# gergely-flamich/compression-without-quantization

Measured on AMD Instinct MI355X. Metric: latent blocks encoded/s at KL=16 bits, higher is better.
Workload: dtype f32

## Files before the change

### compression_without_quantization_amd/_lib.py

```python
import ctypes
import os

_HERE = os.path.dirname(os.path.abspath(__file__))
LIB_PATH = os.environ.get("CWQ_LIB_PATH") or os.path.join(_HERE, "libcwq.so")

c_int = ctypes.c_int
c_i32 = ctypes.c_int32
c_i64 = ctypes.c_int64
c_f32 = ctypes.c_float
c_f64 = ctypes.c_double
c_size = ctypes.c_size_t
c_vp = ctypes.c_void_p
c_str = ctypes.c_char_p


class Options(ctypes.Structure):
    _fields_ = [("prune_mode", ctypes.c_int32), ("reserved", ctypes.c_int32),
                ("eval_start_event", c_vp), ("eval_stop_event", c_vp),
                ("eval_ms_out", ctypes.POINTER(ctypes.c_float)),
                ("item_ready", c_vp)]


c_opts = ctypes.POINTER(Options)

# ... 22 lines not shown
                                          c_i32, c_f32, c_i64, c_vp, c_vp, c_vp, c_size, c_opts,
                                          c_vp]),
    "cwq_greedy_decode": (c_int, [c_vp, c_vp, c_vp, c_vp, c_i64, c_i64, c_i64, c_int, c_int,
                                  c_i32, c_f32, c_i64, c_vp, c_vp]),
    "cwq_greedy_decode_uniform": (c_int, [c_vp, c_vp, c_vp, c_i64, c_i64, c_int, c_int, c_i32,
                                          c_f32, c_i64, c_vp, c_vp]),
    "cwq_block_bits": (c_int, [c_vp, c_vp, c_vp, c_vp, c_i64, c_i64, c_f64, c_int, c_int, c_vp,
                               c_vp, c_vp]),
    "cwq_greedy_encode_uniform_var_workspace_size": (c_size, [c_i64, c_i64]),
    "cwq_greedy_encode_uniform_var": (c_int, [c_vp, c_vp, c_vp, c_vp, c_i64, c_i64, c_vp, c_int,
                                              c_i32, c_f32, c_i64, c_vp, c_vp, c_vp, c_size,
                                              c_opts, c_vp]),
    "cwq_block_bits_csr": (c_int, [c_vp, c_vp, c_vp, c_vp, c_vp, c_i64, c_i64, c_f64, c_int,
                                   c_int, c_int, c_vp, c_vp, c_vp]),
    "cwq_greedy_encode_var_workspace_size": (c_size, [c_i64, c_i64, c_i64, c_int]),
    "cwq_greedy_encode_var": (c_int, [c_vp, c_vp, c_vp, c_vp, c_vp, c_i64, c_i64, c_i64, c_vp,
                                      c_int, c_i32, c_f32, c_i64, c_vp, c_vp, c_vp, c_size,
                                      c_opts, c_vp]),
    "cwq_pack_indices_var_workspace_size": (c_size, [c_i64]),
    "cwq_pack_indices_var": (c_int, [c_vp, c_vp, c_i64, c_int, c_vp, c_i64, c_vp, c_vp, c_size,
                                     c_vp]),
    "cwq_unpack_indices_var": (c_int, [c_vp, c_i64, c_vp, c_i64, c_int, c_vp, c_vp, c_size,
                                       c_vp]),
    "cwq_standardise": (c_int, [c_vp, c_vp, c_vp, c_vp, c_i64, c_vp, c_vp, c_vp]),
    "cwq_kl_normal_normal": (c_int, [c_vp, c_vp, c_vp, c_vp, c_i64, c_vp, c_vp]),
    "cwq_destandardise": (c_int, [c_vp, c_vp, c_vp, c_i64, c_vp, c_vp]),
    "cwq_group_starts": (c_i64, [c_vp, c_i64, c_i64, c_f64, c_vp, c_i64]),
    "cwq_code_grouped_greedy_workspace_size": (c_size, [c_i64, c_int]),
    "cwq_code_grouped_greedy": (c_i64, [c_vp, c_vp, c_vp, c_vp, c_i64, c_int, c_int, c_i32, c_f32,
                                        c_i64, c_f64, c_vp, c_vp, c_i64, c_vp, c_i64, c_vp, c_vp,
                                        c_size, c_opts, c_vp]),
    "cwq_code_grouped_greedy_begin": (c_i64, [c_vp, c_vp, c_vp, c_vp, c_i64, c_int, c_int, c_i32,
                                              c_f32, c_i64, c_f64, c_vp, c_vp, c_i64, c_vp, c_i64,
                                              c_vp, c_vp, c_size, c_opts, c_vp]),
    "cwq_code_grouped_greedy_end": (c_i64, [c_vp, c_i64, c_int, c_int, c_vp, c_i64, c_vp]),
    "cwq_code_grouped_greedy_batch_workspace_size": (c_size, [c_i64, c_i64, c_int]),
    "cwq_code_grouped_greedy_batch_host_workspace_size": (c_size, [c_i64, c_i64, c_int]),
    "cwq_code_grouped_greedy_batch": (c_i64, [c_i64, c_vp, c_vp, c_vp, c_vp, c_vp, c_int, c_int,
                                              c_vp, c_f32, c_i64, c_f64, c_vp, c_vp, c_i64, c_vp,
                                              c_vp, c_i64, c_vp, c_vp, c_size, c_vp, c_size,
                                              c_opts, c_vp]),
    "cwq_importance_workspace_size": (c_size, [c_i64, c_i64]),
    "cwq_importance_encode": (c_int, [c_vp, c_vp, c_vp, c_vp, c_vp, c_vp, c_i64, c_i64, c_i32,
                                      c_i64, c_vp, c_vp, c_vp, c_size, c_opts, c_vp]),
    "cwq_importance_decode": (c_int, [c_vp, c_vp, c_vp, c_vp, c_i64, c_i64, c_i32, c_i64, c_vp,
                                      c_vp]),
    "cwq_importance_group_starts": (c_i64, [c_vp, c_i64, c_i64, c_f64, c_vp, c_i64]),
    "cwq_importance_plan": (c_int, [c_vp, c_vp, c_i64, c_vp]),
    "cwq_code_grouped_importance_workspace_size": (c_size, [c_i64]),
    "cwq_code_grouped_importance": (c_i64, [c_vp, c_vp, c_vp, c_vp, c_i64, c_i32, c_f32, c_i64,
                                            c_f64, c_vp, c_vp, c_vp, c_i64, c_vp, c_vp, c_vp,
                                            c_vp, c_vp, c_size, c_opts, c_vp]),
    "cwq_code_grouped_importance_batch_workspace_size": (c_size, [c_i64, c_i64]),
    "cwq_code_grouped_importance_batch": (c_i64, [c_i64, c_vp, c_vp, c_vp, c_vp, c_vp, c_vp,
                                                  c_f32, c_i64, c_f64, c_vp, c_vp, c_vp, c_i64,
                                                  c_vp, c_vp, c_vp, c_vp, c_vp, c_vp, c_size,
                                                  c_opts, c_vp]),
    "cwq_decode_grouped_greedy_batch_workspace_size": (c_size, [c_i64, c_i64, c_int]),
    "cwq_decode_grouped_greedy_batch_host_workspace_size": (c_size, [c_i64, c_i64, c_int]),
    "cwq_decode_grouped_greedy_batch": (c_i64, [c_i64, c_vp, c_vp, c_vp, c_vp, c_vp, c_vp, c_vp,
                                                c_int, c_int, c_vp, c_f32, c_vp, c_vp, c_vp,
                                                c_size, c_vp, c_size, c_opts, c_vp]),
    "cwq_decode_grouped_importance_batch_workspace_size": (c_size, [c_i64, c_i64]),
    "cwq_decode_grouped_importance_batch_host_workspace_size": (c_size, [c_i64, c_i64]),
    "cwq_decode_grouped_importance_batch": (c_i64, [c_i64, c_vp, c_vp, c_vp, c_vp, c_vp, c_vp,
                                                    c_vp, c_vp, c_vp, c_vp, c_vp, c_size, c_vp,
                                                    c_size, c_opts, c_vp]),
    "cwq_ac_encode": (c_i64, [c_vp, c_i64, c_int, c_vp, c_i64, c_vp, c_i64]),
    "cwq_ac_decode": (c_i64, [c_vp, c_i64, c_int, c_vp, c_i64, c_vp, c_i64]),
    "cwq_elias_delta_encode": (c_i64, [c_vp, c_i64, c_vp, c_i64]),
    "cwq_elias_delta_decode": (c_i64, [c_vp, c_i64, c_i64, c_vp]),
    "cwq_bitcode_to_indices": (c_i64, [c_vp, c_i64, c_int, c_i64, c_vp]),
    "cwq_selftest_bm_tables": (c_int, [ctypes.c_uint32, c_i64, c_vp, c_vp, c_vp, c_vp]),
    "cwq_selftest_screen_tables": (c_int, [ctypes.c_uint32, c_i64, c_vp, c_vp, c_vp, c_vp]),
    "cwq_selftest_logf": (c_int, [c_vp, c_i64, c_vp, c_vp]),
    "cwq_selftest_wave_max": (c_int, [c_vp, c_i64, c_vp, c_vp]),
    "cwq_selftest_div": (c_int, [c_vp, c_vp, c_i64, c_vp, c_vp]),
    "cwq_selftest_encode_rows_wave": (c_int, [c_vp, c_vp, c_vp, c_vp, c_vp, c_i64, c_i64, c_i64,
                                              c_int, c_int, c_i32, c_f32, c_i64, c_vp, c_vp, c_vp,
                                              c_size, c_vp]),
    "cwq_selftest_encode_uniform_tau_guess": (c_int, [c_vp, c_vp, c_vp, c_vp, c_i64, c_i64, c_int,
                                                      c_int, c_i32, c_f32, c_i64, c_vp, c_vp, c_vp,
                                                      c_size, c_opts, c_vp, c_int]),
    "cwq_beam_encode_workspace_size": (c_size, [c_i64, c_i64, c_i64, c_int, c_int]),
    "cwq_beam_encode": (c_int, [c_vp, c_vp, c_vp, c_vp, c_vp, c_i64, c_i64, c_i64, c_int, c_int,
                                c_int, c_i32, c_f32, c_i64, c_vp, c_vp, c_vp, c_vp, c_size, c_opts,
                                c_vp]),
    "cwq_selftest_beam_encode": (c_int, [c_vp, c_vp, c_vp, c_vp, c_vp, c_i64, c_i64, c_i64, c_int,
                                         c_int, c_int, c_i32, c_f32, c_i64, c_vp, c_vp, c_vp, c_vp,
                                         c_size, c_opts, c_vp, c_int]),
    "cwq_beam_encode_var": (c_int, [c_vp, c_vp, c_vp, c_vp, c_vp, c_i64, c_i64, c_i64, c_vp, c_int,
                                    c_int, c_int, c_i32, c_f32, c_i64, c_vp, c_vp, c_vp, c_vp,
                                    c_size, c_opts, c_vp]),
    "cwq_selftest_beam_encode_var": (c_int, [c_vp, c_vp, c_vp, c_vp, c_vp, c_i64, c_i64, c_i64,
                                             c_vp, c_int, c_int, c_int, c_i32, c_f32, c_i64, c_vp,
                                             c_vp, c_vp, c_vp, c_size, c_opts, c_vp, c_int]),
    "cwq_greedy_backfit_workspace_size": (c_size, [c_i64, c_i64, c_i64, c_int]),
    "cwq_greedy_backfit": (c_int, [c_vp, c_vp, c_vp, c_vp, c_vp, c_i64, c_i64, c_i64, c_int, c_int,
                                   c_int, c_i32, c_f32, c_i64, c_vp, c_vp, c_vp, c_vp, c_vp, c_size,
                                   c_opts, c_vp]),
    "cwq_greedy_backfit_var": (c_int, [c_vp, c_vp, c_vp, c_vp, c_vp, c_i64, c_i64, c_i64, c_vp,
                                       c_int, c_int, c_i32, c_f32, c_i64, c_vp, c_vp, c_vp, c_vp,
                                       c_vp, c_size, c_opts, c_vp]),
    "cwq_pln_posterior": (c_int, [c_vp, c_vp, c_vp, c_vp, c_i64, c_f32, c_vp, c_vp, c_vp]),
    "cwq_permute_gather": (c_int, [c_vp, c_i64, c_i64, c_vp, c_vp, c_vp]),
    "cwq_permute_scatter": (c_int, [c_vp, c_i64, c_i64, c_vp, c_vp, c_vp]),
}

TOOL_SIGNATURES = {
    "cwq_debug_prune_stats": (c_int, [c_vp, c_int]),
    "cwq_debug_tile_times": (c_int, [c_vp, c_vp, c_vp, c_int]),
    "cwq_debug_quad_times": (c_int, [c_vp, c_vp, c_int]),
    "cwq_debug_partition_workspace_size": (c_size, [c_i64]),
    "cwq_debug_group_starts_device": (c_i64, [c_vp, c_i64, c_i64, c_f64, c_vp, c_vp, c_size,
                                              c_vp, c_vp]),
}

ABI_VERSION = (0 << 16) | 15

_lib = None


class CwqError(RuntimeError):
    """A libcwq call returned an error code."""


def load():
    global _lib
    if _lib is not None:
        return _lib
    if not os.path.exists(LIB_PATH):
        raise ImportError(
            f"{LIB_PATH} not found: build the HIP extension first "
            "(python -c 'import __graft_entry__ as g; g.build()')")
    lib = ctypes.CDLL(LIB_PATH)
    lib.cwq_version.restype = c_int
    lib.cwq_version.argtypes = []
    ver = lib.cwq_version()
    if ver != ABI_VERSION:
        raise ImportError(f"{LIB_PATH} has ABI version {ver >> 16}.{ver & 0xffff}, these "
                          f"bindings need {ABI_VERSION >> 16}.{ABI_VERSION & 0xffff}: rebuild it")
    for name, (res, args) in list(SIGNATURES.items()) + list(TOOL_SIGNATURES.items()):
        if not hasattr(lib, name):
            if name in TOOL_SIGNATURES:
                continue
            raise ImportError(f"{LIB_PATH} does not export {name}: rebuild it")
        fn = getattr(lib, name)
        fn.restype = res
        fn.argtypes = args
    _lib = lib
    return lib


def check(rc, what):
    if rc < 0:
        msg = load().cwq_last_error().decode("utf-8", "replace")
        raise CwqError(f"{what} failed ({rc}): {msg}")
    return rc
```

### compression_without_quantization_amd/coded_greedy_sampler.py

```python
import array
import concurrent.futures
import ctypes
import functools
import threading
import warnings
import weakref
import time

import numpy as np
import torch

from . import _lib
from .binary_io import bitcode_to_indices, indices_to_bitcode

VERBOSE = True


def _device_of(*xs):
    for x in xs:
        if isinstance(x, torch.Tensor) and x.is_cuda:
            return x.device
    if not torch.cuda.is_available():
        raise RuntimeError("compression_without_quantization_amd needs a ROCm GPU "
                           "(torch.cuda.is_available() is False); there is no CPU path")
    return torch.device("cuda", torch.cuda.current_device())


def _is_float32(x):
    if isinstance(x, torch.Tensor):
        return x.dtype == torch.float32
    return np.asarray(x).dtype == np.float32


def _f32(x, device, what):
    if isinstance(x, torch.Tensor):
        if x.device == device and x.dtype == torch.float32 and x.is_contiguous():
            return x.view(-1)
        t = x
    else:
        t = torch.from_numpy(np.ascontiguousarray(np.asarray(x)))
    if t.dtype != torch.float32:
        raise TypeError(f"{what} must be float32, got {t.dtype}")
    return t.to(device=device).contiguous().reshape(-1)


def _ptr(t):
    return t.data_ptr() if t is not None and t.numel() > 0 else None


def _like_input(t, ref):
    if isinstance(ref, torch.Tensor):
        return t
    return t.cpu().numpy()


class Normal:

    def __init__(self, loc, scale):
        self.loc = loc
        self.scale = scale

    @property
    def dtype(self):
        return self.loc.dtype


def encode_workspace_bytes(nb, total_dims, block_dim=None, max_block_dim=None):
    lib = _lib.load()
    if block_dim is not None:
        return int(lib.cwq_greedy_encode_uniform_workspace_size(int(nb), int(block_dim)))
    mbd = int(total_dims if max_block_dim is None else max_block_dim)
    return int(lib.cwq_greedy_encode_workspace_size(int(nb), int(total_dims), mbd))


def encode_blocks(t_loc, t_scale, p_loc, p_scale, n_bits_per_step, n_steps, seed, rho=1.,
                  block_dim=None, block_off=None, max_block_dim=None, block_id_base=0,
                  out_idx=None, out_sample=None, workspace=None, prune_mode=None,
                  eval_events=None):
    lib = _lib.load()
    dev = _device_of(t_loc, t_scale, p_loc, p_scale)
    tl = _f32(t_loc, dev, "t_loc")
    ts = _f32(t_scale, dev, "t_scale")
    pl = _f32(p_loc, dev, "p_loc")
    ps = _f32(p_scale, dev, "p_scale")
    D = tl.numel()
    if not (ts.numel() == pl.numel() == ps.numel() == D):
        raise ValueError("t_loc, t_scale, p_loc, p_scale must have the same size")
    if (block_dim is None) == (block_off is None):
        raise ValueError("give exactly one of block_dim / block_off")
    if block_dim is not None:
        block_dim = int(block_dim)
        if block_dim < 0 or (block_dim == 0 and D != 0) or (block_dim and D % block_dim):
            raise ValueError(f"D={D} is not a multiple of block_dim={block_dim}")
        nb = D // block_dim if block_dim else 0
        offs = None
    else:
        offs_h = np.asarray(block_off.cpu() if isinstance(block_off, torch.Tensor)
                            else block_off, dtype=np.int64).reshape(-1)
        nb = offs_h.size - 1
        if nb < 0 or offs_h[0] != 0 or offs_h[-1] != D or (np.diff(offs_h) < 0).any():
            raise ValueError("block_off must be non-decreasing from 0 to D")
        if max_block_dim is None:
            max_block_dim = int(np.diff(offs_h).max()) if nb > 0 else 0
        offs = torch.from_numpy(offs_h).to(dev)
    n_steps = int(n_steps)
    if out_idx is None:
        out_idx = torch.empty((nb, n_steps), dtype=torch.int32, device=dev)
    if out_sample is None:
        out_sample = torch.empty(D, dtype=torch.float32, device=dev)
    need = encode_workspace_bytes(nb, D, block_dim if offs is None else None,
                                  None if offs is None else max_block_dim)
    if workspace is None or workspace.numel() < need:
        workspace = torch.empty(max(need, 1), dtype=torch.uint8, device=dev)
    opts = _lib.options(prune_mode, eval_events)
    seed32 = int(np.int32(np.uint32(int(seed) & 0xFFFFFFFF)))
    with torch.cuda.device(dev):
        stream = torch.cuda.current_stream(dev).cuda_stream
        if offs is None:
            rc = lib.cwq_greedy_encode_uniform(
                _ptr(tl), _ptr(ts), _ptr(pl), _ptr(ps), nb, block_dim, int(n_bits_per_step),
                n_steps, seed32, float(rho), int(block_id_base), _ptr(out_idx),
                _ptr(out_sample), workspace.data_ptr(), workspace.numel(), opts, stream)
        else:
            rc = lib.cwq_greedy_encode(
                _ptr(tl), _ptr(ts), _ptr(pl), _ptr(ps), offs.data_ptr(), nb, D,
                int(max_block_dim), int(n_bits_per_step), n_steps, seed32, float(rho),
                int(block_id_base), _ptr(out_idx), _ptr(out_sample), workspace.data_ptr(),
                workspace.numel(), opts, stream)
    _lib.check(rc, "cwq_greedy_encode")
    return out_idx, out_sample


def decode_blocks(idx, p_loc, p_scale, n_bits_per_step, n_steps, seed, rho=1.,
                  block_dim=None, block_off=None, block_id_base=0, out_sample=None):
    lib = _lib.load()
    dev = _device_of(idx, p_loc, p_scale)
    pl = _f32(p_loc, dev, "p_loc")
    ps = _f32(p_scale, dev, "p_scale")
    D = pl.numel()
    if ps.numel() != D:
        raise ValueError("p_loc and p_scale must have the same size")
    it = idx if isinstance(idx, torch.Tensor) else torch.from_numpy(np.asarray(idx))
    it = it.to(device=dev, dtype=torch.int32).contiguous().reshape(-1)
    n_steps = int(n_steps)
    if out_sample is None:
        out_sample = torch.empty(D, dtype=torch.float32, device=dev)
    stream = torch.cuda.current_stream(dev).cuda_stream
    seed32 = int(np.int32(np.uint32(int(seed) & 0xFFFFFFFF)))
    if (block_dim is None) == (block_off is None):
        raise ValueError("give exactly one of block_dim / block_off")
    with torch.cuda.device(dev):
        return _decode_blocks_on(lib, it, pl, ps, D, n_steps, n_bits_per_step, seed32, rho,
                                 block_dim, block_off, block_id_base, out_sample, dev, stream)
# ... 573 lines not shown
```

### compression_without_quantization_amd/csrc/cwq_capi.hip

```cpp
#include <hip/hip_runtime.h>
#include <hsa/hsa.h>
#include <hsa/hsa_ext_amd.h>
#include <stdint.h>
#include <stdarg.h>
#include <stdio.h>
#include <math.h>
#include <string.h>
#include <time.h>
#include <immintrin.h>

#include <algorithm>
#include <atomic>
#include <memory>
#include <condition_variable>
#include <functional>
#include <mutex>
#include <sched.h>
#include <unistd.h>
#include <stdlib.h>
#include <thread>
#include <vector>

#include "../../include/cwq.h"
#include "cwq_debug.h"
// ... 192 lines not shown
      }
    }
  }
  starts[ns++] = D - 1;
  starts[ns++] = D;
  ok();
  return ns;
}

int read_options(const cwq_options* opts, cwq_options* out) {
  const cwq_options def = CWQ_OPTIONS_INIT;
  *out = opts ? *opts : def;
  if (out->prune_mode < 0 || out->prune_mode > 2)
    return fail(CWQ_ERR_INVALID, "cwq_options.prune_mode=%d outside [0, 2]", out->prune_mode);
  if (out->reserved != 0) return fail(CWQ_ERR_INVALID, "cwq_options.reserved must be 0");
  if ((out->eval_start_event == nullptr) != (out->eval_stop_event == nullptr))
    return fail(CWQ_ERR_INVALID, "cwq_options: give both eval events or neither");
  return CWQ_OK;
}

int check_common(int n_bits, int n_steps, int64_t nb) {
  if (n_bits < 0 || n_bits > CWQ_MAX_BITS_PER_STEP)
    return fail(CWQ_ERR_INVALID, "n_bits_per_step=%d outside [0, %d]", n_bits,
                CWQ_MAX_BITS_PER_STEP);
  if (n_steps < 1) return fail(CWQ_ERR_INVALID, "n_steps=%d must be >= 1", n_steps);
  if (nb < 0) return fail(CWQ_ERR_INVALID, "nb=%lld must be >= 0", (long long)nb);
  return CWQ_OK;
}

void fill_encode_args(cwq::EncodeArgs& a, const float* t_loc, const float* t_scale,
                      const float* p_loc, const float* p_scale, const int64_t* block_off,
                      int64_t ud, int64_t nb, int64_t total_dims, int64_t max_d, int n_bits,
                      int n_steps, int32_t seed, float rho, int64_t block_id_base,
                      int32_t* out_idx, float* out_sample, const cwq_options& o,
                      const cwq::EncWs& l, void* w) {
  a.t_loc = t_loc;
  a.t_scale = t_scale;
  a.p_loc = p_loc;
  a.p_scale = p_scale;
  a.block_off = block_off;
  a.ud = ud;
  a.nb = nb;
  a.total_dims = total_dims;
  a.max_d = max_d;
  a.n_cand = (int64_t)1 << n_bits;
  cwq::choose_tiling(nb, a.n_cand, &a.tiles_per_block, &a.cand_per_tile);
  a.n_steps = n_steps;
  a.prune = o.prune_mode;
  a.seed = seed;
  a.rho = rho;
  a.block_id_base = block_id_base;
  a.seeds = nullptr;
  a.out_idx = out_idx;
  a.out_sample = out_sample;
  a.ev_start = o.eval_start_event;
  a.ev_stop = o.eval_stop_event;
  a.keys = at<unsigned long long>(w, l.keys);
  a.tq = at<uint32_t>(w, l.tq);
  a.loc_s = at<float>(w, l.loc_s);
  a.scale_s = at<float>(w, l.scale_s);
  a.lognorm = at<float>(w, l.lognorm);
  a.sab = l.screen ? at<float2>(w, l.sab) : nullptr;
  a.cdim = l.screen ? at<float>(w, l.cdim) : nullptr;
  a.bpre = l.screen ? at<float>(w, l.bpre) : nullptr;
  a.ordu = l.screen ? at<uint32_t>(w, l.ordu) : nullptr;
  a.grp = l.screen ? at<float4>(w, l.grp) : nullptr;
  a.gtau = l.screen ? at<uint32_t>(w, l.gtau) : nullptr;
#ifdef CWQ_NO_RECS
  a.abp = nullptr;
#else
  a.abp = l.recs ? at<float4>(w, l.abp) : nullptr;
#endif
  a.slist = l.screen ? at<uint2>(w, l.slist) : nullptr;
  a.sdmap = l.screen ? at<uint32_t>(w, l.sdmap) : nullptr;
}

int encode_impl(const float* t_loc, const float* t_scale, const float* p_loc,
                const float* p_scale, const int64_t* block_off, int64_t ud, int64_t nb,
                int64_t total_dims, int64_t max_block_dim, int n_bits, int n_steps, int32_t seed,
                float rho, int64_t block_id_base, int32_t* out_idx, float* out_sample,
                void* workspace, size_t workspace_bytes, const cwq_options* opts, void* stream,
                const int32_t* block_seeds = nullptr, float* ds_out = nullptr,
                const float* ds_loc = nullptr, const float* ds_scale = nullptr,
                bool rows_wave = false, int tau_guess = -1) {
  int rc = check_common(n_bits, n_steps, nb);
  if (rc) return rc;
  cwq_options o;
  if ((rc = read_options(opts, &o))) return rc;
  if (total_dims < 0) return fail(CWQ_ERR_INVALID, "total_dims must be >= 0");
  if (nb > 0 && (!out_idx)) return fail(CWQ_ERR_INVALID, "out_idx is null");
  if (total_dims > 0 && (!t_loc || !t_scale || !p_loc || !p_scale || !out_sample))
    return fail(CWQ_ERR_INVALID, "null input/output pointer");
  const cwq::EncWs l = block_off ? cwq::enc_ws_csr(nb, total_dims, max_block_dim)
                                 : cwq::enc_ws_uniform(nb, ud);
  if ((rc = check_ws(workspace, workspace_bytes, l.total, NullWs::TakenIfEmpty))) return rc;
  cwq::EncodeArgs a;
  fill_encode_args(a, t_loc, t_scale, p_loc, p_scale, block_off, ud, nb, total_dims,
                   block_off ? max_block_dim : ud, n_bits, n_steps, seed, rho, block_id_base,
                   out_idx, out_sample, o, l, workspace);
  a.seeds = block_seeds;
  a.ds_out = ds_out;
  a.ds_loc = ds_loc;
  a.ds_scale = ds_scale;
  a.rows_wave = rows_wave;
  a.tau_guess = tau_guess;
  hipError_t e = cwq::launch_encode(a, (hipStream_t)stream);
  if (e != hipSuccess) return hip_fail(e, "cwq_greedy_encode");
  return ok();
}

cwq_options without_events(cwq_options o) {
  o.eval_start_event = o.eval_stop_event = nullptr;
  o.eval_ms_out = nullptr;
  o.item_ready = nullptr;
  return o;
}

struct SortedBlocks {
  float *t_loc, *t_scale, *p_loc, *p_scale, *sample;
  int32_t *seeds, *perm;
  int64_t *soff, *src;
  cwq::BudgetPlan plan;
  uint32_t bad_entries;
};

int sort_blocks(const char* who, const float* const in[4], const int64_t* block_off, int64_t nb,
                int64_t total_dims, int64_t max_block_dim, const int32_t* n_bits, int n_steps,
                int32_t seed, int64_t block_id_base, int prune_mode, void* w,
                const cwq::SortedWs& l, const int32_t* table, int32_t* table_s,
                uint32_t* bad_dev, hipStream_t st, SortedBlocks* s) {
  const bool csr = block_off != nullptr;
  *s = {at<float>(w, l.t_loc),   at<float>(w, l.t_scale), at<float>(w, l.p_loc),
        at<float>(w, l.p_scale), at<float>(w, l.sample),  at<int32_t>(w, l.seeds),
        at<int32_t>(w, l.perm),  at<int64_t>(w, l.soff),  at<int64_t>(w, l.src)};
  uint32_t* counts_dev = at<uint32_t>(w, l.counts);
  cwq::VbcFacts* facts_dev = at<cwq::VbcFacts>(w, l.facts);
  int64_t* roff = at<int64_t>(w, l.roff);
  hipError_t e = cwq::launch_vb_sort(n_bits, nb, s->perm, at<uint32_t>(w, l.hist), counts_dev, st);
  if (e == hipSuccess && csr) {
    e = cwq::launch_vbc_layout(n_bits, block_off, s->perm, nb, counts_dev,
                               at<unsigned long long>(w, l.wgfacts), facts_dev, seed,
                               block_id_base, s->soff, roff, s->src, s->seeds,
                               at<int64_t>(w, l.partial), st);
    if (e == hipSuccess)
      e = cwq::launch_vbc_gather(in[0], in[1], in[2], in[3], s->soff, s->src, nb, total_dims,
                                 s->t_loc, s->t_scale, s->p_loc, s->p_scale, st);
  } else if (e == hipSuccess) {
    e = cwq::launch_vb_gather(in[0], in[1], in[2], in[3], s->perm, nb, max_block_dim, seed,
                              block_id_base, s->t_loc, s->t_scale, s->p_loc, s->p_scale, s->seeds,
                              st);
  }
  if (e == hipSuccess && table)
    e = cwq::launch_vb_gather_table(table, n_bits, s->perm, nb, n_steps, table_s, bad_dev, st);
  if (e != hipSuccess)
    return fail(CWQ_ERR_HIP, "%s (sort / gather): %s", who, hipGetErrorString(e));
  cwq::VbcFacts f;
  uint32_t cb[33] = {0};
  if (csr) {
    e = hipMemcpyAsync(&f, facts_dev, sizeof(f), hipMemcpyDeviceToHost, st);
    if (e == hipSuccess && table)
      e = hipMemcpyAsync(&cb[32], bad_dev, 4, hipMemcpyDeviceToHost, st);
  } else {
    e = hipMemcpyAsync(cb, counts_dev, (table ? 33 : 32) * 4, hipMemcpyDeviceToHost, st);
  }
  if (e == hipSuccess) e = hipStreamSynchronize(st);
  if (e != hipSuccess) return fail(CWQ_ERR_HIP, "%s (facts): %s", who, hipGetErrorString(e));
  if (!csr) f = cwq::uniform_facts(cb, max_block_dim);
  s->bad_entries = cb[32];
  const cwq::BudgetPlan& p = s->plan;
  switch (cwq::budget_plan(f, csr, nb, total_dims, max_block_dim, n_steps, prune_mode, roff,
                           &s->plan)) {
    case cwq::BudgetRefusal::BitsOutOfRange:
      return fail(CWQ_ERR_INVALID, "%u of %lld n_bits values outside [0, %d]", (unsigned)p.got,
                  (long long)p.limit, CWQ_MAX_BITS_PER_STEP);
    case cwq::BudgetRefusal::BadLength:
      return fail(CWQ_ERR_INVALID, "block_off decreases at %lld blocks", (long long)p.got);
    case cwq::BudgetRefusal::TooManyDims:
      return fail(CWQ_ERR_INVALID, "the blocks hold %lld dims, total_dims=%lld", (long long)p.got,
                  (long long)p.limit);
    case cwq::BudgetRefusal::BlockTooLong:
      return fail(CWQ_ERR_INVALID, "a block holds %lld dims, max_block_dim=%lld",
                  (long long)p.got, (long long)p.limit);
    case cwq::BudgetRefusal::None:
      break;
  }
  return CWQ_OK;
}
}

namespace cwq {
int set_error(int code, const char* msg) { return fail(code, "%s", msg); }
}

extern "C" {

int cwq_version(void) { return CWQ_ABI_VERSION; }

const char* cwq_last_error(void) { return g_err; }

int cwq_stateless_normal_sample(const float* loc, const float* scale, int64_t d,
                                int64_t num_samples, int32_t seed, float* out, void* stream) {
  if (d < 0 || num_samples < 0) return fail(CWQ_ERR_INVALID, "negative size");
  if (d * num_samples > 0 && (!loc || !scale || !out))
    return fail(CWQ_ERR_INVALID, "null pointer");
  hipError_t e =
      cwq::launch_stateless_normal_sample(loc, scale, d, num_samples, seed, out, (hipStream_t)stream);
  if (e != hipSuccess) return hip_fail(e, "cwq_stateless_normal_sample");
  return ok();
}

size_t cwq_greedy_encode_workspace_size(int64_t nb, int64_t total_dims, int64_t max_block_dim) {
  if (nb < 0 || total_dims < 0 || max_block_dim < 0) return 0;
  return cwq::enc_ws_csr(nb, total_dims, max_block_dim).total;
}

size_t cwq_greedy_encode_uniform_workspace_size(int64_t nb, int64_t d) {
  if (nb < 0 || d < 0 || (d > 0 && nb > INT64_MAX / d)) return 0;
  return cwq::enc_ws_uniform(nb, d).total;
}

int cwq_greedy_encode(const float* t_loc, const float* t_scale, const float* p_loc,
                      const float* p_scale, const int64_t* block_off, int64_t nb,
                      int64_t total_dims, int64_t max_block_dim, int n_bits_per_step,
                      int n_steps, int32_t seed, float rho, int64_t block_id_base,
                      int32_t* out_idx, float* out_sample, void* workspace,
                      size_t workspace_bytes, const cwq_options* opts, void* stream) {
  if (nb > 0 && !block_off) return fail(CWQ_ERR_INVALID, "block_off is null");
  if (max_block_dim < 0) return fail(CWQ_ERR_INVALID, "max_block_dim must be >= 0");
  return encode_impl(t_loc, t_scale, p_loc, p_scale, block_off, 0, nb, total_dims, max_block_dim,
                     n_bits_per_step, n_steps, seed, rho, block_id_base, out_idx, out_sample,
                     workspace, workspace_bytes, opts, stream);
}

int cwq_greedy_encode_uniform(const float* t_loc, const float* t_scale, const float* p_loc,
                              const float* p_scale, int64_t nb, int64_t d,
                              int n_bits_per_step, int n_steps, int32_t seed, float rho,
                              int64_t block_id_base, int32_t* out_idx, float* out_sample,
                              void* workspace, size_t workspace_bytes, const cwq_options* opts,
                              void* stream) {
  if (d < 0) return fail(CWQ_ERR_INVALID, "d must be >= 0");
  if (nb < 0 || (d > 0 && nb > INT64_MAX / d)) return fail(CWQ_ERR_INVALID, "bad nb");
  return encode_impl(t_loc, t_scale, p_loc, p_scale, nullptr, d, nb, nb * d, d, n_bits_per_step,
                     n_steps, seed, rho, block_id_base, out_idx, out_sample, workspace,
                     workspace_bytes, opts, stream);
}

int cwq_greedy_decode(const int32_t* idx, const float* p_loc, const float* p_scale,
                      const int64_t* block_off, int64_t nb, int64_t total_dims,
                      int64_t max_block_dim, int n_bits_per_step, int n_steps, int32_t seed,
                      float rho, int64_t block_id_base, float* out_sample, void* stream) {
  int rc = check_common(n_bits_per_step, n_steps, nb);
  if (rc) return rc;
  if (nb > 0 && (!block_off || !idx)) return fail(CWQ_ERR_INVALID, "null pointer");
  if (total_dims > 0 && (!p_loc || !p_scale || !out_sample))
    return fail(CWQ_ERR_INVALID, "null pointer");
  (void)max_block_dim;
  hipError_t e = cwq::launch_decode(idx, p_loc, p_scale, block_off, 0, nb, total_dims,
                                    n_bits_per_step,
                                    n_steps, seed, rho, block_id_base, out_sample,
                                    (hipStream_t)stream);
  if (e != hipSuccess) return hip_fail(e, "cwq_greedy_decode");
  return ok();
}

int cwq_greedy_decode_uniform(const int32_t* idx, const float* p_loc, const float* p_scale,
                              int64_t nb, int64_t d, int n_bits_per_step, int n_steps,
                              int32_t seed, float rho, int64_t block_id_base, float* out_sample,
                              void* stream) {
  int rc = check_common(n_bits_per_step, n_steps, nb);
  if (rc) return rc;
  if (d < 0) return fail(CWQ_ERR_INVALID, "d must be >= 0");
  if (nb > 0 && !idx) return fail(CWQ_ERR_INVALID, "null pointer");
  if (nb * d > 0 && (!p_loc || !p_scale || !out_sample))
    return fail(CWQ_ERR_INVALID, "null pointer");
  hipError_t e = cwq::launch_decode(idx, p_loc, p_scale, nullptr, d, nb, nb * d,
                                    n_bits_per_step,
                                    n_steps, seed, rho, block_id_base, out_sample,
                                    (hipStream_t)stream);
  if (e != hipSuccess) return hip_fail(e, "cwq_greedy_decode_uniform");
  return ok();
}

int cwq_standardise(const float* q_loc, const float* q_scale, const float* p_loc,
                    const float* p_scale, int64_t n, float* t_loc, float* t_scale, void* stream) {
  if (n < 0) return fail(CWQ_ERR_INVALID, "negative size");
  if (n > 0 && (!q_loc || !q_scale || !p_loc || !p_scale || !t_loc || !t_scale))
    return fail(CWQ_ERR_INVALID, "null pointer");
  hipError_t e = cwq::launch_standardise(q_loc, q_scale, p_loc, p_scale, n, t_loc, t_scale,
                                         (hipStream_t)stream);
  if (e != hipSuccess) return hip_fail(e, "cwq_standardise");
  return ok();
}

int cwq_kl_normal_normal(const float* q_loc, const float* q_scale, const float* p_loc,
                         const float* p_scale, int64_t n, float* out, void* stream) {
  if (n < 0) return fail(CWQ_ERR_INVALID, "negative size");
  if (n > 0 && (!q_loc || !q_scale || !p_loc || !p_scale || !out))
    return fail(CWQ_ERR_INVALID, "null pointer");
  hipError_t e = cwq::launch_kl(q_loc, q_scale, p_loc, p_scale, n, out, (hipStream_t)stream);
  if (e != hipSuccess) return hip_fail(e, "cwq_kl_normal_normal");
  return ok();
}

int cwq_destandardise(const float* sample, const float* p_loc, const float* p_scale, int64_t n,
                      float* out, void* stream) {
  if (n < 0) return fail(CWQ_ERR_INVALID, "negative size");
  if (n > 0 && (!sample || !p_loc || !p_scale || !out))
    return fail(CWQ_ERR_INVALID, "null pointer");
  hipError_t e =
      cwq::launch_destandardise(sample, p_loc, p_scale, n, out, (hipStream_t)stream);
  if (e != hipSuccess) return hip_fail(e, "cwq_destandardise");
  return ok();
}

namespace {
int check_var_nb(int64_t nb) {
  if (nb < 0 || nb > INT32_MAX)
    return fail(CWQ_ERR_INVALID, "nb=%lld outside [0, 2^31 - 1]", (long long)nb);
  return CWQ_OK;
}
}

int cwq_block_bits(const float* q_loc, const float* q_scale, const float* p_loc,
                   const float* p_scale, int64_t nb, int64_t d, double extra_bits, int min_bits,
                   int max_bits, int32_t* bits_out, float* kl_bits_out, void* stream) {
  if (nb < 0 || d < 0 || (d > 0 && nb > INT64_MAX / d)) return fail(CWQ_ERR_INVALID, "bad nb / d");
  if (min_bits < 0 || max_bits > CWQ_MAX_BITS_PER_STEP || min_bits > max_bits)
// ... 2050 lines not shown
  return D < 0 ? 0 : cwq::part_debug_ws(D).total;
}

int64_t cwq_debug_group_starts_device(const float* kl, int64_t D, int64_t size_threshold,
                                      double n_nats, int64_t* starts, void* workspace,
                                      size_t workspace_bytes, unsigned long long* info_host,
                                      void* stream) {
  if (!kl || !starts || !workspace || !info_host || D < 0)
    return fail(CWQ_ERR_INVALID, "cwq_debug_group_starts_device: bad arguments");
  if (!cwq::partition_applies(D, size_threshold)) return 0;
  const cwq::PartDebugWs l = cwq::part_debug_ws(D);
  if (workspace_bytes < l.total)
    return fail(CWQ_ERR_WORKSPACE, "cwq_debug_group_starts_device: workspace too small");
  hipStream_t s = (hipStream_t)stream;
  unsigned long long* info_d = at<unsigned long long>(workspace, l.info);
  hipError_t e = cwq::launch_partition(kl, D, nullptr, 1, size_threshold, group_thr(n_nats, false),
                                       starts, (int64_t*)(info_d + 8), workspace, info_d, s);
  unsigned long long h[16];
  if (e == hipSuccess)
    e = hipMemcpyAsync(h, info_d, sizeof(h), hipMemcpyDeviceToHost, s);
  if (e == hipSuccess) e = hipStreamSynchronize(s);
  if (e != hipSuccess) return hip_fail(e, "cwq_debug_group_starts_device");
  ok();
  for (int i = 0; i < 8; ++i) info_host[i] = h[i];
  info_host[0] = h[8] - 1;
  info_host[1] = h[9];
  return cwq::partition_fell_back(h) ? 0 : (int64_t)h[8];
}

int cwq_debug_tile_times(unsigned long long* t0, unsigned long long* t1, unsigned int* wg,
                         int n) {
  if (!t0 || !t1 || !wg || n < 0) return fail(CWQ_ERR_INVALID, "cwq_debug_tile_times: bad args");
  const int r = cwq::tile_times(t0, t1, wg, n);
  if (r < 0) return fail(CWQ_ERR_HIP, "cwq_debug_tile_times: symbol copy failed");
  return r;
}

int cwq_debug_quad_times(unsigned long long* t, unsigned int* info, int n) {
  if (!t || !info || n < 0) return fail(CWQ_ERR_INVALID, "cwq_debug_quad_times: bad args");
  const int r = cwq::quad_times(t, info, n);
  if (r < 0) return fail(CWQ_ERR_HIP, "cwq_debug_quad_times: symbol copy failed");
  return r;
}

int cwq_debug_prune_stats(unsigned long long* out72, int flags) {
  if (!out72) return fail(CWQ_ERR_INVALID, "cwq_debug_prune_stats: null output");
  const int r = cwq::prune_stats(out72, flags);
  if (r < 0) return fail(CWQ_ERR_HIP, "cwq_debug_prune_stats: symbol copy failed");
  cwq::set_error(CWQ_OK, "");
  return r;
}

int cwq_selftest_encode_rows_wave(const float* t_loc, const float* t_scale, const float* p_loc,
                                  const float* p_scale, const int64_t* block_off, int64_t nb,
                                  int64_t total_dims, int64_t max_block_dim, int n_bits_per_step,
                                  int n_steps, int32_t seed, float rho, int64_t block_id_base,
                                  int32_t* out_idx, float* out_sample, void* workspace,
                                  size_t workspace_bytes, void* stream) {
  if (nb > 0 && !block_off) return fail(CWQ_ERR_INVALID, "block_off is null");
  if (max_block_dim < 0) return fail(CWQ_ERR_INVALID, "max_block_dim must be >= 0");
  return encode_impl(t_loc, t_scale, p_loc, p_scale, block_off, 0, nb, total_dims, max_block_dim,
                     n_bits_per_step, n_steps, seed, rho, block_id_base, out_idx, out_sample,
                     workspace, workspace_bytes, nullptr, stream, nullptr, nullptr, nullptr,
                     nullptr, true);
}

int cwq_selftest_encode_uniform_tau_guess(const float* t_loc, const float* t_scale,
                                          const float* p_loc, const float* p_scale, int64_t nb,
                                          int64_t d, int n_bits_per_step, int n_steps,
                                          int32_t seed, float rho, int64_t block_id_base,
                                          int32_t* out_idx, float* out_sample, void* workspace,
                                          size_t workspace_bytes, const cwq_options* opts,
                                          void* stream, int guess_mode) {
  if (d < 0) return fail(CWQ_ERR_INVALID, "d must be >= 0");
  if (nb < 0 || (d > 0 && nb > INT64_MAX / d)) return fail(CWQ_ERR_INVALID, "bad nb");
  if (guess_mode < 0 || guess_mode > 2)
    return fail(CWQ_ERR_INVALID, "guess_mode=%d outside [0, 2]", guess_mode);
  return encode_impl(t_loc, t_scale, p_loc, p_scale, nullptr, d, nb, nb * d, d, n_bits_per_step,
                     n_steps, seed, rho, block_id_base, out_idx, out_sample, workspace,
                     workspace_bytes, opts, stream, nullptr, nullptr, nullptr, nullptr,
                     false, guess_mode);
}

namespace {
int beam_impl(const float* t_loc, const float* t_scale, const float* p_loc, const float* p_scale,
              const int64_t* block_off, int64_t nb, int64_t total_dims, int64_t max_block_dim,
              int n_bits, int n_steps, int beam, int32_t seed, float rho, int64_t block_id_base,
              int32_t* out_idx, float* out_sample, float* out_value, void* workspace,
              size_t workspace_bytes, const cwq_options* opts, void* stream, int path,
              const int32_t* n_bits_dev = nullptr, bool var = false) {
  if (var && (n_bits < 0 || n_bits > CWQ_MAX_BITS_PER_STEP))
    return fail(CWQ_ERR_INVALID, "max_bits=%d outside [0, %d]", n_bits, CWQ_MAX_BITS_PER_STEP);
  int rc = check_common(n_bits, n_steps, nb);
  if (rc) return rc;
  cwq_options o;
  if ((rc = read_options(opts, &o))) return rc;
  if (beam < 1 || beam > CWQ_MAX_BEAM)
    return fail(CWQ_ERR_INVALID, "beam=%d outside [1, %d]", beam, CWQ_MAX_BEAM);
  if (((int64_t)beam << n_bits) > (1LL << 31))
    return fail(CWQ_ERR_INVALID, "beam * 2^%s = %lld exceeds 2^31",
                var ? "max_bits" : "n_bits_per_step", (long long)((int64_t)beam << n_bits));
  if (var && nb > 0 && !n_bits_dev) return fail(CWQ_ERR_INVALID, "n_bits is null");
  if (total_dims < 0 || max_block_dim < 0)
    return fail(CWQ_ERR_INVALID, "total_dims and max_block_dim must be >= 0");
  if (path < -1 || path > 3) return fail(CWQ_ERR_INVALID, "path=%d outside [0, 3]", path);
  if (!block_off && nb > 0 && (max_block_dim > INT64_MAX / nb || nb * max_block_dim != total_dims))
    return fail(CWQ_ERR_INVALID, "uniform blocks: total_dims must be nb * max_block_dim");
  if (nb > 0 && !out_idx) return fail(CWQ_ERR_INVALID, "out_idx is null");
  if (total_dims > 0 && (!t_loc || !t_scale || !p_loc || !p_scale || !out_sample))
    return fail(CWQ_ERR_INVALID, "null input/output pointer");
  const cwq::BeamPath plan = cwq::beam_plan(max_block_dim);
  if (path >= 0 && (path & 1) == 0 && plan != cwq::BeamPath::LanePerRow)
    return fail(CWQ_ERR_INVALID, "the lane-per-row kernel takes blocks of at most %d dims",
                CWQ_FUSED_DMAX);
  if ((rc = check_ws(workspace, workspace_bytes,
                     cwq::beam_ws(nb, total_dims, n_steps, beam).total, NullWs::TakenIfEmpty)))
    return rc;
  cwq::BeamArgs a;
  a.t_loc = t_loc;
  a.t_scale = t_scale;
  a.p_loc = p_loc;
  a.p_scale = p_scale;
  a.block_off = block_off;
  a.ud = block_off ? 0 : max_block_dim;
  a.nb = nb;
  a.total_dims = total_dims;
  a.max_d = max_block_dim;
  a.n_bits = n_bits;
  a.n_steps = n_steps;
  a.beam = beam;
  a.seed = seed;
  a.rho = rho;
  a.block_id_base = block_id_base;
  a.out_idx = out_idx;
  a.out_sample = out_sample;
  a.out_value = out_value;
  a.workspace = workspace;
  a.ev_start = o.eval_start_event;
  a.ev_stop = o.eval_stop_event;
  a.path = path < 0 ? plan
                    : ((path & 1) ? cwq::BeamPath::WavePerRow : cwq::BeamPath::LanePerRow);
  a.quarter_tiles = path >= 2;
  a.n_bits_dev = var ? n_bits_dev : nullptr;
  hipError_t e = cwq::launch_beam_encode(a, (hipStream_t)stream);
  if (e != hipSuccess) return hip_fail(e, var ? "cwq_beam_encode_var" : "cwq_beam_encode");
  return ok();
}
}

size_t cwq_beam_encode_workspace_size(int64_t nb, int64_t total_dims, int64_t max_block_dim,
                                      int n_steps, int beam) {
  if (nb < 0 || total_dims < 0 || max_block_dim < 0 || n_steps < 1 || beam < 1 ||
      beam > CWQ_MAX_BEAM)
    return 0;
  return cwq::beam_ws(nb, total_dims, n_steps, beam).total;
}

int cwq_beam_encode(const float* t_loc, const float* t_scale, const float* p_loc,
                    const float* p_scale, const int64_t* block_off, int64_t nb,
                    int64_t total_dims, int64_t max_block_dim, int n_bits_per_step, int n_steps,
                    int beam, int32_t seed, float rho, int64_t block_id_base, int32_t* out_idx,
                    float* out_sample, float* out_value, void* workspace, size_t workspace_bytes,
                    const cwq_options* opts, void* stream) {
  return beam_impl(t_loc, t_scale, p_loc, p_scale, block_off, nb, total_dims, max_block_dim,
                   n_bits_per_step, n_steps, beam, seed, rho, block_id_base, out_idx, out_sample,
                   out_value, workspace, workspace_bytes, opts, stream, -1);
// ... 180 lines not shown
```

### compression_without_quantization_amd/csrc/cwq_kernels.h

```cpp
#pragma once
#include <hip/hip_runtime.h>
#include <stdint.h>

#include "cwq_dispatch.h"
#include "cwq_workspace.h"
#include "cwq_budget_plan.h"

namespace cwq {

int set_error(int code, const char* msg);

__host__ __device__ inline int64_t csr_rec_base(int64_t off) {
  return off + 12 * (off / (CWQ_CSR_LDS_DIMS + 1));
}

struct EncodeArgs {
  const float* t_loc;
  const float* t_scale;
  const float* p_loc;
  const float* p_scale;
  const int64_t* block_off;
  int64_t ud;
  int64_t nb;
  int64_t total_dims;
  int64_t max_d;
  int64_t n_cand;
  int64_t tiles_per_block;
  int64_t cand_per_tile;
  int n_steps;
  int prune;
  int tau_guess = -1;
  int32_t seed;
  float rho;
  int64_t block_id_base;
  const int32_t* seeds;
  int32_t* out_idx;
  float* out_sample;
  unsigned long long* keys;
  uint32_t* tq = nullptr;
  float* loc_s;
  float* scale_s;
  float* lognorm;
  float2* sab;
  float* cdim;
  float* bpre;
  uint32_t* ordu;
  float4* grp;
  uint32_t* gtau;
  float4* abp;
  uint2* slist;
  void* ev_start;
  void* ev_stop;
  const float2* pre_ab = nullptr;
  uint32_t* sdmap = nullptr;
  float* ds_out = nullptr;
  const float* ds_loc = nullptr;
  const float* ds_scale = nullptr;
  bool rows_wave = false;
};

hipStream_t copy_stream(hipStream_t stream, int which);
hipError_t launch_encode(const EncodeArgs& a, hipStream_t stream);
hipError_t launch_decode(const int32_t* idx, const float* p_loc, const float* p_scale,
                         const int64_t* block_off, int64_t ud, int64_t nb, int64_t total_dims,
                         int n_bits,
                         int n_steps, int32_t seed, float rho, int64_t block_id_base,
                         float* out_sample, hipStream_t stream);
__host__ __device__ inline int64_t decode_csr_slots(int64_t d) {
  return d > 0 ? ((d + 3) >> 2) + 1 : 0;
}
hipError_t launch_decode_csr_q4(const int32_t* idx, const int64_t* block_off,
                                const int64_t* slot_off, int64_t nb, int64_t n_slots,
                                const int32_t* block_seeds, int n_bits, int n_steps, float rho,
                                const float* dst_loc, const float* dst_scale, float* out,
                                hipStream_t stream);
hipError_t launch_stateless_normal_sample(const float* loc, const float* scale, int64_t d,
                                          int64_t num_samples, int32_t seed, float* out,
                                          hipStream_t stream);
hipError_t launch_standardise(const float* q_loc, const float* q_scale, const float* p_loc,
                              const float* p_scale, int64_t n, float* t_loc, float* t_scale,
                              hipStream_t stream);
hipError_t launch_kl(const float* q_loc, const float* q_scale, const float* p_loc,
                     const float* p_scale, int64_t n, float* out, hipStream_t stream);
hipError_t launch_destandardise(const float* sample, const float* p_loc, const float* p_scale,
                                int64_t n, float* out, hipStream_t stream);
hipError_t launch_imp_grouped_prep(const float* q_loc, const float* q_scale, const float* p_loc,
                                   const float* p_scale, int64_t n, float limit,
                                   const int64_t* item_off, const int32_t* seed1, int64_t n_items,
                                   int32_t seed1_one, float* t_loc, float* t_scale, uint8_t* keep,
                                   float* zeros, float* ones, float* kl2, float* tsamp,
                                   hipStream_t stream);
hipError_t launch_grouped_prep(const float* q_loc, const float* q_scale, const float* p_loc,
                               const float* p_scale, int64_t n, float* t_loc, float* t_scale,
                               float* kl, float* zeros, float* ones, unsigned long long* zinfo,
                               int nz, hipStream_t stream);

bool partition_applies(int64_t D, int64_t size_threshold);
struct BatchItem {
  int64_t src, rel, go, gs, G, term, dc;
  int64_t pk, ns;
  int32_t seed, pad;
};
static_assert(sizeof(BatchItem) == kBatchItemBytes, "batch_ws sizes the layout table by it");
hipError_t launch_batch_layout(const BatchItem* items, int64_t n_items, const int64_t* dstarts,
                               int64_t* offs, int32_t* seeds, int64_t* pstarts,
                               hipStream_t stream);
hipError_t launch_partition(const float* kl, int64_t D, const int64_t* item_off, int64_t n_items,
                            int64_t size_threshold, float thr, int64_t* starts, int64_t* iinfo,
                            void* ws, unsigned long long* info, hipStream_t stream,
                            bool info_zeroed = false);
bool partition_fell_back(const unsigned long long* info_host);

hipError_t launch_imp_outliers(const float* kl, int64_t n, float limit, float* t_loc,
                               float* t_scale, uint8_t* keep, hipStream_t stream);
hipError_t launch_importance_encode(const float* t_loc, const float* t_scale, const float* p_loc,
                                    const float* p_scale, const int64_t* block_off,
                                    const int64_t* n_samples, int64_t nb, int64_t total_dims,
                                    int32_t seed, int64_t block_id_base,
                                    const int32_t* block_seeds, int allow_screen,
                                    int64_t* out_index, float* out_sample,
                                    void* workspace,
                                    hipStream_t stream, int64_t total_cands = -1,
// ... 118 lines not shown
```

### compression_without_quantization_amd/csrc/cwq_kernels.hip

```cpp
#include <hip/hip_runtime.h>

#include <type_traits>
#include <stdint.h>

#include "cwq_device.h"
#include "cwq_kernels.h"
#include "cwq_refill.h"
#include "cwq_tau_guess.h"

namespace cwq {

__global__ void __launch_bounds__(256) k_prep_dims(
    const float* __restrict__ t_scale, const float* __restrict__ p_loc,
    const float* __restrict__ p_scale, int64_t n, float nst, float sdiv, float rho,
    float* __restrict__ loc_s, float* __restrict__ scale_s, float* __restrict__ lognorm,
    float* __restrict__ out_sample, unsigned long long* __restrict__ keys, int64_t nb) {
  for (int64_t g = blockIdx.x * (int64_t)blockDim.x + threadIdx.x; g < nb;
       g += (int64_t)gridDim.x * blockDim.x)
    keys[g] = 0ull;
  for (int64_t i = blockIdx.x * (int64_t)blockDim.x + threadIdx.x; i < n;
       i += (int64_t)gridDim.x * blockDim.x) {
    float ls, ss;
    shard_consts(p_loc[i], p_scale[i], nst, sdiv, rho, ls, ss);
    loc_s[i] = ls;
    scale_s[i] = ss;
    lognorm[i] = lognorm_of(t_scale[i]);
    out_sample[i] = 0.0f;
  }
}

template <int DC, bool STEP0>
__device__ __forceinline__ float eval_row(const PhiloxStream& st, uint64_t kbase, int64_t d_rt,
                                          int align_rt, const float* __restrict__ loc_s,
                                          const float* __restrict__ scale_s,
                                          const float* __restrict__ mu,
                                          const float* __restrict__ sg,
                                          const float* __restrict__ lognorm,
                                          const float* __restrict__ best,
                                          const double* logtab) {
  return eval_row_f<DC>(st, kbase, d_rt, align_rt, logtab, [&](int64_t e, float zz) -> float {
    float s = scale_s[e] * zz;
    s = loc_s[e] + s;
    const float tv = STEP0 ? s : best[e] + s;
    return log_prob(tv, mu[e], sg[e], lognorm[e]);
  });
}

template <int DC, bool STEP0>
__global__ void __launch_bounds__(256) k_encode_eval(
    const float* __restrict__ t_loc, const float* __restrict__ t_scale,
    const float* __restrict__ loc_s, const float* __restrict__ scale_s,
    const float* __restrict__ lognorm, const float* __restrict__ best,
    const int64_t* __restrict__ block_off, int64_t ud, int64_t ntiles, int64_t tiles_per_block,
    int64_t cand_per_tile, int64_t n_cand, SeedSpec sd, int32_t step,
    unsigned long long* __restrict__ keys) {
  __shared__ double logtab[32];
  __shared__ unsigned long long wkey[4];
  fill_logtab(logtab);
  const uint32_t wv = wave_id();
  const uint32_t lane = threadIdx.x & 63u;

  for (int64_t tile = blockIdx.x; tile < ntiles; tile += gridDim.x) {
    const int64_t g = tile / tiles_per_block;
    const int64_t tt = tile - g * tiles_per_block;
    const BlockSpan sp = block_span(block_off, ud, g);
    const int64_t n0 = tt * cand_per_tile;
    const int64_t n1 = (n0 + cand_per_tile < n_cand) ? n0 + cand_per_tile : n_cand;
    const PhiloxStream st =
        generate_key(step_seed(sd.of(g), step), 42);
    const int align = (int)(((uint64_t)(n0 + wv) * (uint64_t)sp.d) & 3u);

    uint64_t bestk = 0;
    for (int64_t n = n0 + 4 * (int64_t)lane + wv; n < n1; n += 256) {
      const float v = eval_row<DC, STEP0>(st, (uint64_t)n * (uint64_t)sp.d, sp.d, align,
                                          loc_s + sp.off, scale_s + sp.off, t_loc + sp.off,
                                          t_scale + sp.off, lognorm + sp.off,
                                          STEP0 ? nullptr : best + sp.off, logtab);
      const uint64_t k = argmax_key(v, (uint32_t)n);
      bestk = k > bestk ? k : bestk;
    }
    bestk = wave_max_u64(bestk);
    if (lane == 0) wkey[wv] = bestk;
    __syncthreads();
    if (threadIdx.x == 0) {
      uint64_t m = wkey[0];
      for (int i = 1; i < 4; ++i) m = wkey[i] > m ? wkey[i] : m;
      if (m) atomicMax(&keys[g], (unsigned long long)m);
    }
    __syncthreads();
  }
}

constexpr float kPruneC1 = 0x1p-14f;
#ifndef CWQ_PRUNE_MIN_WAVES
#define CWQ_PRUNE_MIN_WAVES 6
#endif
#ifndef CWQ_XCD_BALANCE
#define CWQ_XCD_BALANCE 1
#endif
#ifndef CWQ_TAU_SHARE_MASK
#define CWQ_TAU_SHARE_MASK 7u
#endif
#ifndef CWQ_CSR_TAU_SHARE_MASK
#define CWQ_CSR_TAU_SHARE_MASK 15u
#endif
#ifndef CWQ_SURVIVOR_CAP
#define CWQ_SURVIVOR_CAP 1024
#endif
#ifndef CWQ_LINKED_VISIT
#define CWQ_LINKED_VISIT 1
#endif
#ifndef CWQ_FOLD_ROUND0
#define CWQ_FOLD_ROUND0 1
#endif
#ifndef CWQ_BORROW_REFILL
#define CWQ_BORROW_REFILL 1
#endif
#ifndef CWQ_POOL_RANGE_SKIP
#define CWQ_POOL_RANGE_SKIP 1
#endif
#ifndef CWQ_PARK_COMPLETE
#define CWQ_PARK_COMPLETE 1
#endif
#ifndef CWQ_PARK_MIN_ROWS
#define CWQ_PARK_MIN_ROWS 8192
#endif
#ifndef CWQ_PARK_MIN_D
#define CWQ_PARK_MIN_D 16
#endif
#if CWQ_PARK_COMPLETE && !(CWQ_LINKED_VISIT && CWQ_BORROW_REFILL)
#error "CWQ_PARK_COMPLETE needs CWQ_LINKED_VISIT and CWQ_BORROW_REFILL"
#endif
#ifndef CWQ_SHARE_UNROLL
#define CWQ_SHARE_UNROLL 8
#endif
#ifndef CWQ_PARK_LOOK_MASK
#define CWQ_PARK_LOOK_MASK CWQ_TAU_SHARE_MASK
#endif
#if CWQ_SHARE_UNROLL != 1 && CWQ_SHARE_UNROLL != 2 && CWQ_SHARE_UNROLL != 4 && CWQ_SHARE_UNROLL != 8
#error "CWQ_SHARE_UNROLL is 1, 2, 4 or 8"
#endif

template <bool STEP0>
__device__ __forceinline__ float cand_diff(float z, float ls, float ss, float mu, float bb) {
  const float s = shard_sample(ls, ss, z);
  const float tv = STEP0 ? s : bb + s;
  return tv - mu;
}
__device__ __forceinline__ float lp_from_z(float z, float cc) {
  const float u = -0.5f * (z * z);
  return u - cc;
}


struct VisitRec {
  float4 sa, sb;
  uint32_t add[2];
  int bk;
  int next;
};
static_assert(sizeof(VisitRec) == 48, "VisitRec: 48 bytes");

template <int D, bool STEP0>
__device__ __forceinline__ float score_rows_wave(
    const PhiloxStream& st, const uint32_t* rows, uint32_t cnt, const float* __restrict__ loc_s,
    const float* __restrict__ scale_s, const float* __restrict__ mu,
    const float* __restrict__ sg, const float* __restrict__ lognorm,
    const float* __restrict__ best, const double* logtab, float* buf, uint32_t lane) {
  constexpr uint32_t G = D / 4;
  const uint32_t r = lane / G, u = lane - r * G;
  if (r < cnt) {
    const F4 z = normal4_dev(st, (uint64_t)rows[r] * G + u, logtab);
#pragma unroll
    for (int t = 0; t < 4; ++t) {
      const uint32_t j = 4u * u + (uint32_t)t;
      const float zz = t == 0 ? z.a : (t == 1 ? z.b : (t == 2 ? z.c : z.d));
      float v = scale_s[j] * zz;
      v = loc_s[j] + v;
      const float tv = STEP0 ? v : best[j] + v;
      buf[r * D + j] = log_prob(tv, mu[j], sg[j], lognorm[j]);
    }
  }
  __builtin_amdgcn_fence(__ATOMIC_SEQ_CST, "wavefront");
  __builtin_amdgcn_wave_barrier();
  float acc = 0.0f;
  const uint32_t fr = lane >> 3;
  if (fr < cnt)
    for (uint32_t e = lane & 7u; e < (uint32_t)D; e += 8u) acc = acc + buf[fr * D + e];
  __builtin_amdgcn_fence(__ATOMIC_SEQ_CST, "wavefront");
  __builtin_amdgcn_wave_barrier();
  float p[8];
#pragma unroll
  for (int l = 0; l < 8; ++l) p[l] = __shfl(acc, (int)((lane & ~7u) + (uint32_t)l), 64);
  return eigen_fold8(p, 0.0f);
}

#ifdef CWQ_TILE_TIMES
constexpr int kTileTimes = 1 << 18;
__device__ unsigned long long g_tile_t0[kTileTimes], g_tile_t1[kTileTimes];
__device__ unsigned int g_tile_wg[kTileTimes];
#endif
#ifdef CWQ_PRUNE_STATS
__device__ unsigned long long g_prune_stats[72];
constexpr int kDbgBlocks = 1 << 20;
__device__ unsigned long long g_dbg_best[kDbgBlocks];
__device__ int g_seed_tau;
#endif

struct TauGuessWaveDims {
  float w, b2;
  int d;
  __device__ __forceinline__ int count() const { return d; }
  template <class F>
  __device__ __forceinline__ cwq::TauGuessSums sum(F f) const {
    cwq::TauGuessSums o = f(w, b2);
#pragma unroll
    for (int sh = 32; sh >= 1; sh >>= 1) {
      o.k += __shfl_xor(o.k, sh, 64);
      o.k1 += __shfl_xor(o.k1, sh, 64);
      o.k2 += __shfl_xor(o.k2, sh, 64);
    }
    return o;
  }
};
__device__ __forceinline__ uint64_t sgpr_pair_uniform(uint64_t v) {
  const uint32_t lo = (uint32_t)__builtin_amdgcn_readfirstlane((int)(uint32_t)v);
  const uint32_t hi = (uint32_t)__builtin_amdgcn_readfirstlane((int)(uint32_t)(v >> 32));
  return ((uint64_t)hi << 32) | lo;
}
constexpr float kTauForceRetry = -2.0f;
__device__ __forceinline__ float tau_guess_of(float qm, float As, float Pq) {
  if (qm == kTauForceRetry) return 3.402823466e+38f;
  if (!(qm >= 0.0f)) return -__builtin_inff();
  const float tg = cwq::screen_row_lower(-qm, cwq::kScreenC2, As, Pq);
  return tg == tg ? tg : -__builtin_inff();
}

template <class F, uint32_t... I>
__device__ __forceinline__ void unroll_each(F& f, std::integer_sequence<uint32_t, I...>) {
  (f(std::integral_constant<uint32_t, I>{}, std::integral_constant<uint32_t, (uint32_t)sizeof...(I)>{}), ...);
}

template <int D, bool STEP0, bool INTER, bool PARK>
__global__ void __launch_bounds__(256, CWQ_PRUNE_MIN_WAVES) k_encode_prune(
    const float* __restrict__ t_loc, const float* __restrict__ t_scale,
    const float* __restrict__ loc_s, const float* __restrict__ scale_s,
    const float* __restrict__ lognorm, const float* __restrict__ best, int64_t ntiles,
    int64_t tiles_per_block, int64_t cand_per_tile, int64_t n_cand, SeedSpec sd, int32_t step,
    int allow_screen, unsigned long long* __restrict__ keys, int64_t tail_from, int tail_div,
    uint32_t* __restrict__ tq) {
  static_assert(D % 8 == 0 && D >= 8 && D <= 64, "pruned path: D % 8 == 0, D <= 64");
  static_assert(!PARK || CWQ_PARK_COMPLETE, "PARK instances exist in CWQ_PARK_COMPLETE builds only");
  constexpr int G = D / 4;
  constexpr int NF = STEP0 ? 6 : 7;
  constexpr int RW = (64 / G) < 8 ? (64 / G) : 8;
  __shared__ double logtab[32];
  __shared__ float4 cst[G * NF];
  constexpr int NREC = CWQ_FOLD_ROUND0 ? 4 : 1;
  constexpr int RPW = G + (PARK ? 1 : 0);
  __shared__ VisitRec vrec[NREC * RPW];
  __shared__ uint32_t w0g_cell[4];
  __shared__ int2 meta[G];
  __shared__ float rowbuf[4][RW * D];
  __shared__ float dscore[D];
  __shared__ float dA[D];
  __shared__ float dC[D];
  __shared__ float gscore[G];
  __shared__ int gpos[G];
  __shared__ float lowc;
  __shared__ float scr_a, scr_pq;
  __shared__ float tau_cell;
  __shared__ float tau_seed_cell;
  __shared__ float qm_cell;
  __shared__ uint32_t sq_cnt;
  __shared__ uint32_t sq_n[CWQ_SURVIVOR_CAP];
  __shared__ float sq_ub[CWQ_SURVIVOR_CAP];
  __shared__ unsigned long long wkey[4];
  __shared__ uint32_t s_next;
#ifdef CWQ_PRUNE_STATS
  __shared__ uint32_t s_ps[72];
  for (int i = threadIdx.x; i < 72; i += blockDim.x) s_ps[i] = 0u;
#endif
  fill_logtab(logtab);
  const uint32_t wv = wave_id();
  const uint32_t lane = threadIdx.x & 63u;

  constexpr bool inter = INTER;
  const int64_t nbt = INTER ? ntiles / tiles_per_block : 0;
  auto next_tile = [&](int64_t cur) -> int64_t {
    if (tq == nullptr) return cur + gridDim.x;
    __syncthreads();
    if (threadIdx.x == 0) s_next = gridDim.x + atomicAdd(tq, 1u);
    __syncthreads();
    return (int64_t)s_next;
  };
  for (int64_t tile = blockIdx.x; tile < ntiles; tile = next_tile(tile)) {
    uint32_t tid = threadIdx.x;
    asm volatile("" : "+v"(tid));
#ifdef CWQ_TILE_TIMES
    if (tid == 0 && tile < kTileTimes) {
      g_tile_t0[tile] = __builtin_amdgcn_s_memrealtime();
      const uint32_t xcc = (uint32_t)__builtin_amdgcn_s_getreg((20) | (0 << 6) | ((4 - 1) << 11));
      g_tile_wg[tile] = (xcc << 24) | (blockIdx.x & 0xffffffu);
    }
#endif
    int64_t tord = tile;
    const int64_t treg = inter ? nbt * tail_from : 0;
    if (inter && CWQ_XCD_BALANCE && tq == nullptr && tile < treg && (treg & 7) == 0 &&
        (gridDim.x & 7u) == 0)
      tord = (tile & 7) * (treg >> 3) + (tile >> 3);
    const int64_t g = inter ? tord % nbt : tile / tiles_per_block;
    const int64_t tt = inter ? tord / nbt : tile - g * tiles_per_block;
    const int64_t off = g * D;
    int64_t n0, csz;
    if (tt < tail_from) {
      n0 = tt * cand_per_tile;
      csz = cand_per_tile;
    } else {
      csz = cand_per_tile / tail_div;
      n0 = tail_from * cand_per_tile + (tt - tail_from) * csz;
    }
    const int64_t n1 = (n0 + csz < n_cand) ? n0 + csz : n_cand;
    if (n0 >= n1) continue;
    const PhiloxStream st =
        generate_key(step_seed(sd.of(g), step), 42);

    if (tid < D) {
      const int j = tid;
      const float ls = loc_s[off + j], ss = scale_s[off + j], mu = t_loc[off + j];
      const float rs = 1.0f / t_scale[off + j];
      const float m = (STEP0 ? ls : best[off + j] + ls) - mu;
      float e = 0.5f * (ss * ss + m * m) * (rs * rs);
      dscore[j] = (e == e) ? e : -1.0f;
    }
    __syncthreads();
    if (tid < G) {
      const int q = tid;
      gscore[q] = ((dscore[4 * q] + dscore[4 * q + 1]) + dscore[4 * q + 2]) + dscore[4 * q + 3];
    }
    __syncthreads();
    if (tid < G) {
      const int q = tid;
      const float sq = gscore[q];
      int r = 0;
      for (int q2 = 0; q2 < G; ++q2) {
        const float s2 = gscore[q2];
        r += (s2 > sq || (s2 == sq && q2 < q)) ? 1 : 0;
      }
      gpos[q] = r;
      meta[r].x = q;
#pragma unroll
      for (int w = 0; w < NREC; ++w) {
        const uint32_t wg = (uint32_t)(n0 + (int64_t)w * ((n1 - n0 + 3) / 4)) * (uint32_t)G;
        const uint64_t add =
            CWQ_FOLD_ROUND0 ? cwq::philox_round0_addend(wg + (uint32_t)q) : (uint64_t)q;
        VisitRec& v = vrec[w * RPW + r];
        v.add[0] = (uint32_t)add;
        v.add[1] = (uint32_t)(add >> 32);
        v.next = (r + 1 < G || PARK) ? (w * RPW + r + 1) * (int)sizeof(VisitRec) : 0;
      }
    }
    if (PARK && tid >= 64 && tid < 64 + NREC) {
      VisitRec& v = vrec[(tid - 64) * RPW + G];
      v.sa = float4{0.f, 0.f, 0.f, 0.f};
      v.sb = float4{0.f, 0.f, 0.f, 0.f};
      v.add[0] = 0u;
      v.add[1] = 0u;
      v.bk = (int)f2u(__builtin_inff());
      v.next = (int)((tid - 64) * RPW + G) * (int)sizeof(VisitRec);
    }
    __syncthreads();
    int den_ok = 1, scr_ok = 1;
    if (tid < D) {
      const int j = tid, k = gpos[j >> 2], w = j & 3;
      float fj[7];
      const float sgj = t_scale[off + j];
      fj[0] = loc_s[off + j];
      fj[1] = scale_s[off + j];
      fj[2] = t_loc[off + j];
      fj[3] = sgj;
      fj[4] = lognorm[off + j];
      fj[5] = 1.0f / sgj;
      fj[6] = STEP0 ? 0.0f : best[off + j];
      float* c = reinterpret_cast<float*>(cst);
#pragma unroll
      for (int f = 0; f < NF; ++f) c[(k * NF + f) * 4 + w] = fj[f];
      den_ok = markstein_ok_den(sgj) ? 1 : 0;
      const ScreenDim o = screen_dim<STEP0>(fj[0], fj[1], fj[2], sgj, fj[4], fj[6]);
#pragma unroll
      for (int c = 0; c < NREC; ++c) {
        float* sc = reinterpret_cast<float*>(&vrec[c * RPW + k]);
        sc[w] = o.sa;
        sc[4 + w] = o.sb;
      }
      dA[j] = o.A;
      dC[j] = o.C;
      scr_ok = o.ok ? 1 : 0;
    }
    const bool fastdiv = __syncthreads_and(den_ok) != 0;
    const bool scr_all = __syncthreads_and(scr_ok) != 0;
    const bool screen = (allow_screen & 1) && scr_all;
    if (wv == 1u) {
      const int gmode = (allow_screen >> 1) & 3;
      float qm = cwq::kTauNoGuess;
      if (screen && gmode == 1) {
        float w = 0.0f, b2 = 0.0f;
        if (lane < (uint32_t)D) {
          const float* sc = reinterpret_cast<const float*>(&vrec[lane >> 2]);
          const float al = sc[lane & 3u] * (float)(1.0 / cwq::kSqrt2Ln2);
          const float be = sc[4u + (lane & 3u)];
          w = al * al;
          b2 = be * be;
        }
        qm = cwq::tau_guess_q(TauGuessWaveDims{w, b2, D}, n1 - n0, cwq::kTauGuessM);
      } else if (screen && gmode == 2) {
        qm = kTauForceRetry;
      }
      if (lane == 0) qm_cell = qm;
    }
    if (tid <= G + 1) {
      const int kb = tid;
      const float* c = reinterpret_cast<const float*>(cst);
      double rf = 0.0, kk = 0.0, asum = 0.0, msum = 0.0, kall = 0.0, cvis = 0.0, a2 = 0.0,
             amax = 0.0;
#pragma unroll 1
      for (int p = 0; p < D; ++p) {
        const double mj = -(double)c[((p >> 2) * NF + 4) * 4 + (p & 3)];
        const double aj = __builtin_fabs(mj);
        asum += aj;
        msum += mj;
        kall += aj + mj;
        if (p >= 4 * kb) {
          rf += mj + 0x1p-17 * aj;
        } else {
          kk += aj + mj;
          if (screen) cvis += (double)dC[(meta[p >> 2].x << 2) + (p & 3)];
        }
        if (screen && kb == G + 1) {
          const double av = (double)dA[p];
          a2 += av * av;
          amax = av > amax ? av : amax;
        }
      }
      const double marg = 0x1p-20 * (__builtin_fabs(rf) + asum) + 0x1p-126;
      const double sl = 0x1p-14 * (__builtin_fabs(msum) + asum + kall) + 0x1p-126;
      if (kb <= G) {
        const float bk = screen ? round_up_f32(msum + cvis * (1.0 + 0x1p-20) + sl)
                                : round_up_f32(rf + 0x1p-14 * kk + marg);
        if (kb >= 1) {
          meta[kb - 1].y = (int)f2u(bk);
#pragma unroll
          for (int c = 0; c < NREC; ++c) vrec[c * RPW + kb - 1].bk = (int)f2u(bk);
        }
        if (kb == G) lowc = round_up_f32(0x1p-14 * kk + marg);
      } else if (screen) {
        scr_a = screen_as(msum, sl, a2);
        scr_pq = screen_pq(amax, D);
      }
      if (kb == 0) {
        float t0 = -__builtin_inff();
        if (inter) {
          const unsigned long long kv =
              __hip_atomic_load(&keys[g], __ATOMIC_RELAXED, __HIP_MEMORY_SCOPE_AGENT);
          if ((uint32_t)(kv >> 32) > kArgmaxClampOrd) t0 = unord_f32((uint32_t)(kv >> 32));
        }
#ifdef CWQ_PRUNE_STATS
        if (g_seed_tau && g < kDbgBlocks && (g_dbg_best[g] >> 32) > kArgmaxClampOrd)
          t0 = unord_f32((uint32_t)(g_dbg_best[g] >> 32));
#endif
        tau_cell = t0;
        tau_seed_cell = t0;
        sq_cnt = 0u;
      }
    }
    __syncthreads();
    const float lc = lowc;
#ifdef CWQ_PRUNE_STATS
    const float tau_seed = tau_cell;
#endif
    const float sA = scr_a, sPq = scr_pq;

    const int64_t per_wave = (n1 - n0 + 3) / 4;
    const int64_t w0 = n0 + (int64_t)wv * per_wave;
    const int64_t w1 = (w0 + per_wave < n1) ? w0 + per_wave : n1;
// ... 99 lines not shown
        } else {
          box_muller_dev(x.x, x.y, logtab, z0, z1);
          box_muller_dev(x.z, x.w, logtab, z2, z3);
          const float4* cq = cst + kp * NF;
          const float4 ls = cq[0], ss = cq[1], mu = cq[2], sg = cq[3], cc = cq[4], ry = cq[5];
          const float4 bb = STEP0 ? float4{0.f, 0.f, 0.f, 0.f} : cq[6];
          const float d0 = cand_diff<STEP0>(z0, ls.x, ss.x, mu.x, bb.x);
          const float d1 = cand_diff<STEP0>(z1, ls.y, ss.y, mu.y, bb.y);
          const float d2 = cand_diff<STEP0>(z2, ls.z, ss.z, mu.z, bb.z);
          const float d3 = cand_diff<STEP0>(z3, ls.w, ss.w, mu.w, bb.w);
          float y0 = div_rn_markstein(d0, sg.x, ry.x);
          float y1 = div_rn_markstein(d1, sg.y, ry.y);
          float y2 = div_rn_markstein(d2, sg.z, ry.z);
          float y3 = div_rn_markstein(d3, sg.w, ry.w);
          const bool ok = fastdiv & markstein_ok4(d0, d1, d2, d3);
          if (__builtin_expect(__ballot(!ok) != 0ull, 0)) {
            if (!ok) {
              y0 = d0 / sg.x;
              y1 = d1 / sg.y;
              y2 = d2 / sg.z;
              y3 = d3 / sg.w;
            }
          }
          s = s + lp_from_z(y0, cc.x);
          s = s + lp_from_z(y1, cc.y);
          s = s + lp_from_z(y2, cc.z);
          s = s + lp_from_z(y3, cc.w);
          upper = (s + __builtin_fabsf(s) * kPruneC1) + u2f((uint32_t)mt.y);
        }
        if constexpr (LINKED)
          kp = kp_next;
        else
          kp += KS;
        const bool complete =
            PARKED ? false : (LINKED ? (kp == 0u) : (kp == kb + KS * (uint32_t)G));
        const bool below = upper < tau;
        const bool reach = SCREEN ? !below : (upper >= tau);
#ifdef CWQ_PRUNE_STATS
        const bool complete_st =
            PARKED ? (kp == kb + KS * (uint32_t)G && kp_was != kb + KS * (uint32_t)G) : complete;
        const bool prune = !complete_st && below;
        const uint32_t k = (LINKED && complete_st) ? (uint32_t)G : (kp - kb) / KS;
#endif
        const bool done = complete || below || !active;
        const uint64_t m_cpl = __builtin_amdgcn_ballot_w64(complete);
        const uint64_t m_below = __builtin_amdgcn_fcmpf(upper, tau, 4 );
        uint64_t m = m_cpl | m_below;
        if constexpr (!FAST) m |= __builtin_amdgcn_read_exec() & ~m_act;
        uint64_t m_keep =
            m_cpl & (FAST ? ~0ull : m_act) &
            (SCREEN ? ~m_below : (uint64_t)__builtin_amdgcn_fcmpf(upper, tau, 3 ));
        constexpr bool LOOK_HERE =
            PARKED && (C + 1u == UU || (LOOK_MASK + 1u <= UU && ((C + 1u) & LOOK_MASK) == 0u));
        if constexpr (!PARKED)
          asm volatile("" : "+s"(m), "+s"(m_keep));
        else if constexpr (!FAST || LOOK_HERE)
          asm volatile("" : "+s"(m));
        auto keep_rows = [&](const uint64_t mk) {
          const bool keep = CWQ_BORROW_REFILL ? ((mk >> lane) & 1ull) != 0ull
                                              : (complete && active && reach);
          float lower;
          if constexpr (SCREEN)
            lower = screen_row_lower(s, kScreenC2, sA, sPq);
          else
            lower = (s - __builtin_fabsf(s) * kPruneC1) - lc;
          if constexpr (PARKED) {
            uint32_t kf = (uint32_t)G - 1u;
            asm volatile("" : "+v"(kf));
            upper = screen_row_upper(s, kScreenC1, u2f((uint32_t)meta[kf].y));
          }
          tau = tau_raise_wave(tau, keep, lower);
          if (__builtin_expect(keep && upper >= tau, 0)) {
            uint32_t ngc = ng;
            asm volatile("" : "+v"(ngc));
            const uint32_t n =
                (*const_cast<const volatile uint32_t*>(&w0g_cell[wv]) + ngc) / (uint32_t)G;
#ifdef CWQ_PRUNE_STATS
            atomicAdd(&s_ps[66], 1u);
#endif
            const uint32_t slot = atomicAdd(&sq_cnt, 1u);
            if (slot < CWQ_SURVIVOR_CAP) {
              sq_n[slot] = (uint32_t)n;
              sq_ub[slot] = upper;
            } else {
#ifdef CWQ_PRUNE_STATS
              atomicAdd(&g_prune_stats[69], 1ull);
#endif
              const float v = eval_row<D, STEP0>(st, (uint64_t)n * D, D, 0, loc_s + off,
                                                 scale_s + off, t_loc + off, t_scale + off,
                                                 lognorm + off, STEP0 ? nullptr : best + off, logtab);
              const uint64_t kv = argmax_key(v, (uint32_t)n);
              bestk = kv > bestk ? kv : bestk;
            }
          }
        };
        if constexpr (!PARKED) {
          if (__builtin_expect(m_keep != 0ull, 0)) keep_rows(m_keep);
        } else {
          if (share_due) tau = tau_share_wave(&tau_cell, tau);
          if (cwq::unroll_due<LOOK_MASK, UU, C>(iter)) {
            const uint64_t m_park = __builtin_amdgcn_uicmp(kp, kb + KS * (uint32_t)G, 32 ) &
                                    (FAST ? ~0ull : m_act) & ~m_below;
            if (__builtin_expect(m_park != 0ull, 0)) keep_rows(m_park);
            m |= m_park;
          }
        }
#ifdef CWQ_PRUNE_STATS
        const bool act_l = ((m_act >> lane) & 1ull) != 0ull;
        if (act_l && (complete_st || prune)) atomicAdd(&s_ps[k], 1u);
        if (act_l && complete_st) atomicAdd(&s_ps[65], 1u);
#endif
        uint64_t m_pool;
        if constexpr (CWQ_BORROW_REFILL) {
          asm volatile(
              "s_mov_b64 exec, %[m]\n\t"
              "v_subrev_co_u32 %[ng], vcc, %[c], %[ng]\n\t"
              "v_mov_b32 %[kp], %[kb]\n\t"
              "v_mov_b32 %[s], 0\n\t"
              "s_mov_b64 exec, -1\n\t"
              "s_and_b64 %[mp], vcc, %[m]\n\t"
              "s_or_b64 %[left], %[left], %[mp]\n\t"
              "s_and_b64 %[mp], %[left], %[m]"
              : [ng] "+v"(ng), [kp] "+v"(kp), [s] "+v"(s), [mp] "=&s"(m_pool),
                [left] "+s"(left)
              : [m] "s"(m), [c] "n"(64 * G), [kb] "s"(kb)
              : "vcc", "scc");
          left = sgpr_pair_uniform(left);
          m_pool = sgpr_pair_uniform(m_pool);
        } else {
          if (done) {
            asm volatile("" : "+v"(ng));
            ng += 64u * (uint32_t)G;
            kp = kb;
            s = 0.0f;
          }
          m_pool = 0ull;
        }
        if (!PARKED && share_due) {
          tau = tau_share_wave(&tau_cell, tau);
        }
        if constexpr (CWQ_BORROW_REFILL) {
          if (FAST ? __builtin_expect(m_pool != 0ull, 0) : (m_pool != 0ull)) {
#ifdef CWQ_PRUNE_STATS
            if (lane == 0) atomicAdd(&s_ps[70], 1u);
#endif
            const uint32_t rank = __builtin_amdgcn_mbcnt_hi(
                (uint32_t)(m_pool >> 32), __builtin_amdgcn_mbcnt_lo((uint32_t)m_pool, 0u));
            asm volatile(
                "s_mov_b64 exec, %[mp]\n\t"
                "v_mad_u32_u24 %[ng], %[rank], %[g], %[wn]\n\t"
                "s_mov_b64 exec, -1"
                : [ng] "+v"(ng)
                : [mp] "s"(m_pool), [rank] "v"(rank), [g] "n"(G), [wn] "s"(wnext_g));
            const uint32_t want = wnext_g + (uint32_t)__builtin_popcountll(m_pool) * (uint32_t)G;
            if constexpr (FAST) {
              wnext_g = want;
            } else if (CWQ_POOL_RANGE_SKIP && want <= ng_end) {
              wnext_g = want;
              m_act |= m_pool;
            } else {
              wnext_g = want < ng_end ? want : ng_end;
              m_act = __builtin_amdgcn_uicmp(ng, ng_end, 36 );
            }
          }
        } else {
          m_pool = m & __builtin_amdgcn_uicmp(ng, ng_stat, 35 );
          if (m_pool != 0ull) {
#ifdef CWQ_PRUNE_STATS
            if (lane == 0) atomicAdd(&s_ps[70], 1u);
#endif
            const uint32_t rank = __builtin_amdgcn_mbcnt_hi(
                (uint32_t)(m_pool >> 32), __builtin_amdgcn_mbcnt_lo((uint32_t)m_pool, 0u));
            if (done && ng >= ng_stat) ng = wnext_g + rank * (uint32_t)G;
            wnext_g += (uint32_t)__builtin_popcountll(m_pool) * (uint32_t)G;
            wnext_g = wnext_g < ng_end ? wnext_g : ng_end;
            active = ng < ng_end;
            m_act = __builtin_amdgcn_ballot_w64(active);
          }
        }
      };
      constexpr std::integral_constant<uint32_t, 0u> c0{};
      constexpr std::integral_constant<uint32_t, 1u> u1{};
      if constexpr (U > 1u) {
        while (m_act == ~0ull && wnext_g + cwq::unroll_trip_rows(U) * (uint32_t)G <= ng_end)
          unroll_each(body, std::make_integer_sequence<uint32_t, U>{});
      }
      while (m_act != 0ull) body(c0, u1);
    };
#ifdef CWQ_PRUNE_STATS
    if (screen && tid == 0) atomicAdd(&g_prune_stats[67], 1ull);
#endif
    float tau_final;
    if (screen) {
      for (;;) {
        pass(std::true_type{});
        tau_share_wave(&tau_cell, tau);
        __syncthreads();
        tau_final = tau_cell;
        const float tg = tau_guess_of(qm_cell, sA, sPq);
        const float seed = INTER ? tau_seed_cell : -__builtin_inff();
        const bool held = tau_final > tg || seed >= tg;
        if (__builtin_amdgcn_readfirstlane(held ? 1 : 0) != 0) break;
        __syncthreads();
        if (tid == 0) {
          tau_cell = seed;
          sq_cnt = 0u;
          qm_cell = cwq::kTauNoGuess;
#ifdef CWQ_PRUNE_STATS
          atomicAdd(&g_prune_stats[51], 1ull);
#endif
        }
        __syncthreads();
        tau = (INTER && CWQ_TAU_FROM_KEYS) ? seed : -__builtin_inff();
      }
    } else {
      pass(std::false_type{});
      tau_share_wave(&tau_cell, tau);
      __syncthreads();
      tau_final = tau_cell;
    }
    const uint32_t nsurv = sq_cnt < CWQ_SURVIVOR_CAP ? sq_cnt : CWQ_SURVIVOR_CAP;
    const uint32_t nsurv_u = (uint32_t)__builtin_amdgcn_readfirstlane((int)nsurv);
    const uint32_t sl = tid & 63u;
    for (uint32_t c0 = wv * 64u; c0 < nsurv_u; c0 += 256u) {
      const uint32_t i = c0 + sl;
      const bool q = i < nsurv_u && sq_ub[i] >= tau_final;
      const uint32_t nn = i < nsurv_u ? sq_n[i] : 0u;
      const uint64_t qm = __builtin_amdgcn_ballot_w64(q);
      if (qm == 0ull) continue;
#ifdef CWQ_PRUNE_STATS
      if (q) atomicAdd(&g_prune_stats[68], 1ull);
#endif
      const uint32_t qr = __builtin_amdgcn_mbcnt_hi((uint32_t)(qm >> 32),
                                                    __builtin_amdgcn_mbcnt_lo((uint32_t)qm, 0u));
      __builtin_amdgcn_fence(__ATOMIC_SEQ_CST, "wavefront");
      __builtin_amdgcn_wave_barrier();
      if (q) sq_n[c0 + qr] = nn;
      __builtin_amdgcn_fence(__ATOMIC_SEQ_CST, "wavefront");
      __builtin_amdgcn_wave_barrier();
      const uint32_t qn = (uint32_t)__builtin_popcountll(qm);
      for (uint32_t b = 0; b < qn; b += (uint32_t)RW) {
        const uint32_t cnt = qn - b < (uint32_t)RW ? qn - b : (uint32_t)RW;
        const float v = score_rows_wave<D, STEP0>(
            st, sq_n + c0 + b, cnt, loc_s + off, scale_s + off, t_loc + off, t_scale + off,
            lognorm + off, STEP0 ? nullptr : best + off, logtab, rowbuf[wv], sl);
        if ((sl & 7u) == 0u && (sl >> 3) < cnt) {
          const uint64_t kv = argmax_key(v, sq_n[c0 + b + (sl >> 3)]);
          bestk = kv > bestk ? kv : bestk;
        }
      }
    }

    bestk = wave_max_u64(bestk);
    if (lane == 0) wkey[wv] = bestk;
    __syncthreads();
    if (tid == 0) {
      uint64_t mk = wkey[0];
      for (int i = 1; i < 4; ++i) mk = wkey[i] > mk ? wkey[i] : mk;
      if (mk) atomicMax(&keys[g], (unsigned long long)mk);
#ifdef CWQ_PRUNE_STATS
      if (!g_seed_tau && g < kDbgBlocks) g_dbg_best[g] = mk;
#endif
#ifdef CWQ_TILE_TIMES
      if (tile < kTileTimes) g_tile_t1[tile] = __builtin_amdgcn_s_memrealtime();
#endif
    }
#ifdef CWQ_PRUNE_STATS
    if (tid < 72) {
      if (s_ps[tid]) atomicAdd(&g_prune_stats[tid], (unsigned long long)s_ps[tid]);
      s_ps[tid] = 0u;
    }
#endif
    __syncthreads();
  }
}

__device__ __forceinline__ double block_sum_d(double v, double* red) {
  red[threadIdx.x] = v;
  __syncthreads();
  for (int w = 128; w > 0; w >>= 1) {
    if ((int)threadIdx.x < w) red[threadIdx.x] += red[threadIdx.x + w];
    __syncthreads();
  }
  const double r = red[0];
  __syncthreads();
  return r;
}

__host__ __device__ __forceinline__ int64_t csr_cls_stride(int64_t d) { return (d + 6) / 4 + 1; }
constexpr int64_t kCsrSortUnits = 2048;

template <bool STEP0>
__global__ void __launch_bounds__(256) k_csr_prep(
    const float* __restrict__ t_loc, const float* __restrict__ t_scale,
    const float* __restrict__ loc_s, const float* __restrict__ scale_s,
    const float* __restrict__ lognorm, const float* __restrict__ best,
    const int64_t* __restrict__ block_off, int64_t ud, int64_t nb, float2* __restrict__ sab,
    float* __restrict__ cdim, float* __restrict__ bpre, uint32_t* __restrict__ ordu,
    float4* __restrict__ grp, uint32_t* __restrict__ gtau, float4* __restrict__ abp,
    int64_t lds_dims, int64_t coop_min_d) {
  __shared__ double red[5][4];
  __shared__ double wscan[4];
  __shared__ double ucs[256];
  __shared__ unsigned long long skey[kCsrSortUnits];
  const int tid = threadIdx.x;
  const int lane = tid & 63, wv = tid >> 6;
  const bool lead = blockIdx.y == 0;
  for (int64_t g = blockIdx.x; g < nb; g += gridDim.x) {
    const BlockSpan sp = block_span(block_off, ud, g);
    const int64_t off = sp.off, d = sp.d;
    ScreenSums u;
    float2* sabg = sab + off + 8 * g + 4;
    float* cg = cdim + off;
    if (lead && tid < 8) {
      if (tid < 4) sabg[tid - 4] = float2{0.f, 0.f};
      sabg[d + tid] = float2{0.f, 0.f};
    }
    for (int64_t j = tid; j < d; j += 256) {
      const ScreenDim o =
          screen_dim<STEP0>(loc_s[off + j], scale_s[off + j], t_loc[off + j], t_scale[off + j],
                            lognorm[off + j], STEP0 ? 0.0f : best[off + j]);
      sabg[j] = float2{o.sa, o.sb};
      cg[j] = o.C;
      u.add(o);
    }
    u.sm = wave_sum_f64(u.sm);
    u.sa = wave_sum_f64(u.sa);
    u.sk = wave_sum_f64(u.sk);
    u.s2 = wave_sum_f64(u.s2);
    u.mx = wave_max_f64(u.mx);
    if (lane == 0) {
      red[0][wv] = u.sm;
      red[1][wv] = u.sa;
      red[2][wv] = u.sk;
      red[3][wv] = u.s2;
      red[4][wv] = u.mx;
    }
    __threadfence_block();
    const bool all_ok = __syncthreads_and(u.ok) != 0;
    ScreenSums S;
    S.sm = ((red[0][0] + red[0][1]) + red[0][2]) + red[0][3];
    S.sa = ((red[1][0] + red[1][1]) + red[1][2]) + red[1][3];
    S.sk = ((red[2][0] + red[2][1]) + red[2][2]) + red[2][3];
    S.s2 = ((red[3][0] + red[3][1]) + red[3][2]) + red[3][3];
    S.mx = red[4][0];
    for (int w = 1; w < 4; ++w) S.mx = red[4][w] > S.mx ? red[4][w] : S.mx;
    const bool coop_blk = d >= coop_min_d;
    const ScreenBlock bc =
        screen_block_consts(S, d, coop_blk ? 16.0 + (double)d / 64.0 : (double)d);
    const double SM = S.sm, sl = bc.sl;
    const int64_t reg = off + 12 * g, cs = csr_cls_stride(d);
    const bool recs = abp != nullptr && d > lds_dims;
    auto sab_at = [&](int64_t j) {
      const unsigned long long v = __hip_atomic_load(
          reinterpret_cast<unsigned long long*>(sabg + j), __ATOMIC_RELAXED,
          __HIP_MEMORY_SCOPE_AGENT);
// ... 2003 lines not shown
                                                       float* __restrict__ out) {
  for (int64_t i = blockIdx.x * (int64_t)blockDim.x + threadIdx.x; i < n;
       i += (int64_t)gridDim.x * blockDim.x)
    out[i] = logf_full(x[i], kLogTabConst);
}

__global__ void __launch_bounds__(256) k_selftest_div(const float* __restrict__ a,
                                                      const float* __restrict__ b, int64_t n,
                                                      float* __restrict__ out) {
  for (int64_t i = blockIdx.x * (int64_t)blockDim.x + threadIdx.x; i < n;
       i += (int64_t)gridDim.x * blockDim.x) {
    const float y = 1.0f / b[i];
    out[i] = div_rn_markstein(a[i], b[i], y);
  }
}


static SeedSpec seeds_of(const EncodeArgs& a) {
  return SeedSpec{a.seed, a.block_id_base, a.seeds};
}

static bool aligned16(const void* a, const void* b, const void* c) {
  return (((uintptr_t)a | (uintptr_t)b | (uintptr_t)c) & 15u) == 0;
}

hipError_t launch_prep_dims(const float* t_scale, const float* p_loc, const float* p_scale,
                            int64_t n, int n_steps, float rho, float* loc_s, float* scale_s,
                            float* lognorm, float* out_sample, unsigned long long* keys,
                            int64_t nb, hipStream_t stream) {
  if (n <= 0 && nb <= 0) return hipSuccess;
  const float nst = (float)n_steps;
  const float sdiv = (float)__builtin_sqrt((double)n_steps);
  hipLaunchKernelGGL(k_prep_dims, dim3(grid_for(n > nb ? n : nb, 256, 65536)), dim3(256), 0,
                     stream, t_scale, p_loc, p_scale, n, nst, sdiv, rho, loc_s, scale_s, lognorm,
                     out_sample, keys, nb);
  return hipGetLastError();
}

template <int DC, bool STEP0>
static void launch_eval_t(const EncodeArgs& a, int step, hipStream_t stream) {
  const int64_t ntiles = a.nb * a.tiles_per_block;
  const unsigned grid = (unsigned)(ntiles < (1LL << 30) ? ntiles : (1LL << 30));
  hipLaunchKernelGGL((k_encode_eval<DC, STEP0>), dim3(grid), dim3(256), 0, stream, a.t_loc,
                     a.t_scale, a.loc_s, a.scale_s, a.lognorm, a.out_sample, a.block_off, a.ud,
                     ntiles, a.tiles_per_block, a.cand_per_tile, a.n_cand, seeds_of(a),
                     step, a.keys);
}

static int prune_screen_arg(const EncodeArgs& a) {
  const int scr = a.prune >= 2 ? 1 : 0;
  const int gm = a.tau_guess >= 0 ? (a.tau_guess & 3) : scr;
  return scr | (gm << 1);
}

template <int D, bool STEP0>
static void launch_prune_t(const EncodeArgs& a, int step, hipStream_t stream) {
#ifndef CWQ_PRUNE_GRID
#define CWQ_PRUNE_GRID (256 * 6 * 256)
#endif
  constexpr int64_t kPruneGrid = CWQ_PRUNE_GRID;
  const int64_t ntiles = a.nb * a.tiles_per_block;
#ifndef CWQ_TILE_INTERLEAVE
#define CWQ_TILE_INTERLEAVE 1
#endif
#ifndef CWQ_SEED_LOG2
#define CWQ_SEED_LOG2 0
#endif
#ifndef CWQ_SEED_TILE
#define CWQ_SEED_TILE 4096
#endif
#ifndef CWQ_SEED_MIN_TPB
#define CWQ_SEED_MIN_TPB 2
#endif
  const int64_t seed_n = CWQ_SEED_LOG2 > 0 ? ((int64_t)1 << CWQ_SEED_LOG2) : 0;
  const bool seeded = CWQ_TILE_INTERLEAVE && seed_n > 0 && a.tiles_per_block >= CWQ_SEED_MIN_TPB &&
                      a.n_cand >= 4 * seed_n;
  if (seeded) {
    const int64_t cpt_s = seed_n < CWQ_SEED_TILE ? (seed_n > 0 ? seed_n : 1) : CWQ_SEED_TILE;
    const int64_t nt_s = a.nb * (seed_n / cpt_s);
    hipLaunchKernelGGL((k_encode_prune<D, STEP0, true, false>),
                       dim3((unsigned)(nt_s < kPruneGrid ? nt_s : kPruneGrid)), dim3(256), 0,
                       stream, a.t_loc, a.t_scale, a.loc_s, a.scale_s, a.lognorm, a.out_sample,
                       nt_s, seed_n / cpt_s, cpt_s, seed_n, seeds_of(a), step,
                       prune_screen_arg(a), a.keys, seed_n / cpt_s, 1, nullptr);
  }
#ifndef CWQ_TILE_QUEUE
#define CWQ_TILE_QUEUE 1
#endif
#ifndef CWQ_QUEUE_GRID
#define CWQ_QUEUE_GRID 1536
#endif
#ifndef CWQ_QUEUE_MIN_CPT
#define CWQ_QUEUE_MIN_CPT 4096
#endif
  uint32_t* tq = nullptr;
  if (CWQ_TILE_QUEUE && a.tq != nullptr && ntiles < (1LL << 31) &&
      a.cand_per_tile >= CWQ_QUEUE_MIN_CPT && ntiles > CWQ_QUEUE_GRID) {
    if (hipMemsetAsync(a.tq, 0, sizeof(uint32_t), stream) == hipSuccess) tq = a.tq;
  }
  auto qgrid = [&](int64_t nt) -> unsigned {
    const int64_t cap = tq ? (int64_t)CWQ_QUEUE_GRID : kPruneGrid;
    return (unsigned)(nt < cap ? nt : cap);
  };
  const int64_t tile_rows = a.cand_per_tile < a.n_cand ? a.cand_per_tile : a.n_cand;
  auto with_park = [&](auto launch) {
    if constexpr (CWQ_PARK_COMPLETE && D >= CWQ_PARK_MIN_D) {
      if (tile_rows * D >= (int64_t)CWQ_PARK_MIN_ROWS * 32) return launch(std::true_type{});
    }
    return launch(std::false_type{});
  };
  if (CWQ_TILE_INTERLEAVE && (a.tiles_per_block > 1 || seeded)) {
#ifndef CWQ_TAIL_SPLIT
#define CWQ_TAIL_SPLIT 4
#endif
    const int64_t tpb = a.tiles_per_block;
    int64_t from = tpb, div = 1;
    if (CWQ_TAIL_SPLIT > 1 && tpb >= 2 && a.cand_per_tile % (256 * CWQ_TAIL_SPLIT) == 0) {
      div = CWQ_TAIL_SPLIT;
      int64_t L = (2 * 1536 + div * a.nb - 1) / (div * a.nb);
      L = L < tpb / 2 ? L : tpb / 2;
      from = tpb - L;
    }
    const int64_t tpb2 = from + (tpb - from) * div;
    const int64_t nt2 = a.nb * tpb2;
    with_park([&](auto park) {
      hipLaunchKernelGGL((k_encode_prune<D, STEP0, true, decltype(park)::value>),
                         dim3(qgrid(nt2)), dim3(256), 0,
                         stream, a.t_loc, a.t_scale, a.loc_s, a.scale_s, a.lognorm, a.out_sample,
                         nt2, tpb2, a.cand_per_tile, a.n_cand, seeds_of(a), step,
                         prune_screen_arg(a), a.keys, from, (int)div, tq);
    });
  } else {
    with_park([&](auto park) {
      hipLaunchKernelGGL((k_encode_prune<D, STEP0, false, decltype(park)::value>),
                         dim3(qgrid(ntiles)), dim3(256), 0,
                         stream, a.t_loc, a.t_scale, a.loc_s, a.scale_s, a.lognorm, a.out_sample,
                         ntiles, a.tiles_per_block, a.cand_per_tile, a.n_cand, seeds_of(a), step,
                         prune_screen_arg(a), a.keys, a.tiles_per_block, 1, tq);
    });
  }
}

template <bool STEP0>
static void launch_prune_csr(const EncodeArgs& a, bool coop, int step, hipStream_t stream) {
  int64_t tpb, max_tpb;
  if (coop) {
    tpb = (CWQ_CSR_COOP_TILES + a.nb - 1) / a.nb;
    max_tpb = a.n_cand / CWQ_CSR_COOP_TILE > 1 ? a.n_cand / CWQ_CSR_COOP_TILE : 1;
  } else {
    tpb = (CWQ_CSR_TILES + a.nb - 1) / a.nb;
    max_tpb = a.n_cand / CWQ_CSR_TILE > 1 ? a.n_cand / CWQ_CSR_TILE : 1;
  }
  tpb = tpb < max_tpb ? tpb : max_tpb;
  const int64_t cpt = (a.n_cand + tpb - 1) / tpb;
  tpb = (a.n_cand + cpt - 1) / cpt;
#if CWQ_COOP_CLASS_TILES
  if (coop && tpb >= 4) tpb = (tpb + 3) & ~(int64_t)3;
#endif
  const int64_t ntiles = a.nb * tpb;
  const int64_t coop_min_d = coop ? (int64_t)CWQ_CSR_COOP_MIN_D : INT64_MAX;
#ifndef CWQ_PREP_SPLIT_MAX_NB
#define CWQ_PREP_SPLIT_MAX_NB 256
#endif
  const unsigned cls_wgs = a.nb <= CWQ_PREP_SPLIT_MAX_NB ? 4 : 1;
  hipLaunchKernelGGL((k_csr_prep<STEP0>), dim3(grid_for(a.nb, 1, 65536), cls_wgs), dim3(256), 0,
                     stream, a.t_loc, a.t_scale, a.loc_s, a.scale_s, a.lognorm, a.out_sample,
                     a.block_off, a.ud, a.nb, a.sab, a.cdim, a.bpre, a.ordu, a.grp, a.gtau,
                     a.abp, (int64_t)CWQ_CSR_LDS_DIMS, coop_min_d);
  constexpr int64_t kGrid = 1 << 20;
  const unsigned grid = (unsigned)(ntiles < kGrid ? ntiles : kGrid);
  if (coop)
    hipLaunchKernelGGL((k_encode_prune_csr<STEP0, true>), dim3(grid), dim3(256), 0, stream,
                       a.t_loc, a.t_scale, a.loc_s, a.scale_s, a.lognorm, a.out_sample,
                       a.block_off, a.ud, ntiles, tpb, cpt, a.n_cand, seeds_of(a),
                       step, (const float2*)a.sab, (const float*)a.bpre,
                       (const uint32_t*)a.ordu, (const float4*)a.grp, a.gtau, a.keys,
                       coop_min_d, (const float4*)a.abp);
  else
    hipLaunchKernelGGL((k_encode_prune_csr<STEP0, false>), dim3(grid), dim3(256), 0, stream,
                       a.t_loc, a.t_scale, a.loc_s, a.scale_s, a.lognorm, a.out_sample,
                       a.block_off, a.ud, ntiles, tpb, cpt, a.n_cand, seeds_of(a),
                       step, (const float2*)a.sab, (const float*)a.bpre,
                       (const uint32_t*)a.ordu, (const float4*)a.grp, a.gtau, a.keys,
                       coop_min_d, (const float4*)a.abp);
}

template <bool STEP0>
static void launch_small_pipe(const EncodeArgs& a, int step, hipStream_t stream) {
  SmallRec* rec = (SmallRec*)a.slist;
  float2* pab = const_cast<float2*>(a.pre_ab);
  const float nst = (float)a.n_steps;
  const float sdiv = (float)__builtin_sqrt((double)a.n_steps);
  const unsigned pgrid = grid_for(a.nb, kSmallPrepBlocks, 1u << 31);
  if (STEP0)
    hipLaunchKernelGGL(k_small_prep1<true>, dim3(pgrid), dim3(CWQ_PREP1_THREADS), 0, stream, a.t_loc,
                       a.t_scale, a.p_loc, a.p_scale, nst, sdiv, a.rho, a.loc_s, a.scale_s,
                       a.lognorm, a.out_sample, a.block_off, a.ud, a.nb, seeds_of(a), step,
                       pab, rec, a.sdmap);
  else
    hipLaunchKernelGGL(k_small_prep1<false>, dim3(pgrid), dim3(CWQ_PREP1_THREADS), 0, stream, a.t_loc,
                       a.t_scale, a.p_loc, a.p_scale, nst, sdiv, a.rho, a.loc_s, a.scale_s,
                       a.lognorm, a.out_sample, a.block_off, a.ud, a.nb, seeds_of(a), step,
                       pab, rec, a.sdmap);
  const int64_t nu = a.nb;
  for (int64_t u0 = 0; u0 < nu; u0 += (int64_t)1 << 30)
    hipLaunchKernelGGL((k_small_one<STEP0>),
                       dim3((unsigned)(nu - u0 < (1LL << 30) ? nu - u0 : (1LL << 30))),
                       dim3(64), 0, stream, a.t_loc, a.t_scale, a.loc_s, a.scale_s, a.lognorm,
                       a.out_sample, rec, a.pre_ab, a.nb, u0, a.n_cand, step, a.n_steps,
                       a.out_idx);
  const unsigned dgrid = grid_for(a.total_dims > a.nb ? a.total_dims : a.nb, 256, 16384);
  hipLaunchKernelGGL((k_small_finalize<STEP0>), dim3(dgrid), dim3(256), 0, stream, a.loc_s,
                     a.scale_s, rec, a.sdmap, a.out_idx, step, a.n_steps, a.block_off, a.ud,
                     a.nb, a.out_sample, step == a.n_steps - 1 ? a.ds_out : nullptr, a.ds_loc,
                     a.ds_scale);
}

template <bool STEP0>
static void launch_small_three(const EncodeArgs& a, int step, hipStream_t stream) {
  const int64_t ntiles = a.nb * a.tiles_per_block;
  hipLaunchKernelGGL((k_small_prep<STEP0>), dim3(grid_for(a.nb, 4 * 64, 16384)), dim3(256), 0,
// ... 141 lines not shown
};
thread_local ForkStreams tl_fork[kMaxDevices];
ForkStreams* fork_streams(hipStream_t stream) {
  int dev = 0;
  if (hipStreamGetDevice(stream, &dev) != hipSuccess || dev < 0 || dev >= kMaxDevices)
    return nullptr;
  ForkStreams& f = tl_fork[dev];
  if (!f.ok) {
    int cur = 0;
    if (hipGetDevice(&cur) != hipSuccess) return nullptr;
    if (cur != dev && hipSetDevice(dev) != hipSuccess) return nullptr;
    bool good = true;
    int made_s = 0, made_e = 0, made_c = 0;
    for (int i = 0; i < kMaxSplit && good; ++i) {
      good = hipStreamCreateWithFlags(&f.s[i], hipStreamNonBlocking) == hipSuccess;
      made_s += good;
      good = good && hipEventCreateWithFlags(&f.join[i], hipEventDisableTiming) == hipSuccess;
      made_e += good;
    }
    for (int i = 0; i < 2 && good; ++i) {
      good = hipStreamCreateWithFlags(&f.cp[i], hipStreamNonBlocking) == hipSuccess;
      made_c += good;
    }
    good = good && hipEventCreateWithFlags(&f.fork, hipEventDisableTiming) == hipSuccess;
    if (!good) {
      for (int i = 0; i < made_s; ++i) (void)hipStreamDestroy(f.s[i]);
      for (int i = 0; i < made_e; ++i) (void)hipEventDestroy(f.join[i]);
      for (int i = 0; i < made_c; ++i) (void)hipStreamDestroy(f.cp[i]);
    }
    if (cur != dev) (void)hipSetDevice(cur);
    if (!good) return nullptr;
    f.ok = true;
  }
  return &f;
}
}

hipStream_t copy_stream(hipStream_t stream, int which) {
  ForkStreams* f = fork_streams(stream);
  return f && which >= 0 && which < 2 ? f->cp[which] : nullptr;
}

hipError_t launch_encode(const EncodeArgs& a_in, hipStream_t stream) {
  hipError_t e;
  EncodeArgs a = a_in;
  a.pre_ab = a.sab;
  const EncodeShape shape = shape_of(a);
  const EncodePlan plan = encode_plan(shape);
  const bool screened = plan.path == EncodePath::CsrPruned ||
                        plan.path == EncodePath::SmallPipe || plan.path == EncodePath::SmallThree;
  if (screened && !(a.sab && a.cdim && a.bpre && a.ordu && a.grp && a.gtau && a.slist && a.sdmap))
    return hipErrorInvalidValue;
  if (plan.self_finalizing)
    e = hipSuccess;
  else
    e = launch_prep_dims(a.t_scale, a.p_loc, a.p_scale, a.total_dims, a.n_steps, a.rho, a.loc_s,
                         a.scale_s, a.lognorm, a.out_sample, a.keys, a.nb, stream);
  if (e != hipSuccess) return e;
  if (a.nb == 0) return hipSuccess;
  const bool ds_after = a.ds_out != nullptr && !plan.self_finalizing;
  auto ds = [&]() -> hipError_t {
    if (!ds_after) return hipSuccess;
    return launch_destandardise(a.out_sample, a.ds_loc, a.ds_scale, a.total_dims, a.ds_out,
                                stream);
  };
  const int k = encode_fork_parts(shape, a.n_steps);
  ForkStreams* f = k > 1 ? fork_streams(stream) : nullptr;
  if (f == nullptr) {
    if ((e = encode_steps(a, stream, true)) != hipSuccess) return e;
    return ds();
  }
  if (a.ev_start && (e = hipEventRecord((hipEvent_t)a.ev_start, stream)) != hipSuccess) return e;
  if ((e = hipEventRecord(f->fork, stream)) != hipSuccess) return e;
  int forked = 0;
  for (int i = 0; i < k && e == hipSuccess; ++i) {
    const int64_t g0 = a.nb * i / k, g1 = a.nb * (i + 1) / k;
    EncodeArgs p = a;
    p.block_off = a.block_off + g0;
    p.nb = g1 - g0;
    p.block_id_base = a.block_id_base + g0;
    if (a.seeds) p.seeds = a.seeds + g0;
    p.keys = a.keys + g0;
    if (a.tq) p.tq = a.tq + i;
    p.out_idx = a.out_idx + g0 * a.n_steps;
    if (a.sab) p.sab = a.sab + 8 * g0;
    if (a.bpre) p.bpre = a.bpre + 12 * g0;
    if (a.ordu) p.ordu = a.ordu + 12 * g0;
    if (a.grp) p.grp = a.grp + g0;
    if (a.gtau) p.gtau = a.gtau + g0 * CWQ_CSR_GTAU_STRIDE;
    if (a.slist) p.slist = a.slist + CWQ_SLIST_PER_BLOCK * g0;
    if ((e = hipStreamWaitEvent(f->s[i], f->fork, 0)) != hipSuccess) break;
    forked = i + 1;
    e = encode_steps(p, f->s[i], false);
  }
  for (int i = 0; i < forked; ++i) {
    hipError_t ej = hipEventRecord(f->join[i], f->s[i]);
    if (ej == hipSuccess) ej = hipStreamWaitEvent(stream, f->join[i], 0);
    if (ej != hipSuccess) {
      (void)hipStreamSynchronize(f->s[i]);
      if (e == hipSuccess) e = ej;
    }
  }
  if (e != hipSuccess) return e;
  if (a.ev_stop && (e = hipEventRecord((hipEvent_t)a.ev_stop, stream)) != hipSuccess) return e;
  return ds();
}

hipError_t launch_decode(const int32_t* idx, const float* p_loc, const float* p_scale,
                         const int64_t* block_off, int64_t ud, int64_t nb, int64_t total_dims,
                         int n_bits,
                         int n_steps, int32_t seed, float rho, int64_t block_id_base,
                         float* out_sample, hipStream_t stream) {
  const DecodePlan p = decode_plan(DecodeShape{block_off != nullptr, ud, nb, total_dims, n_steps,
                                               aligned16(p_loc, p_scale, out_sample)});
  if (p.workgroups == 0) return hipSuccess;
  const float nst = (float)n_steps;
  const float sdiv = (float)__builtin_sqrt((double)n_steps);
  switch (p.kernel) {
    case DecodeKernel::Q4Glds:
      hipLaunchKernelGGL(k_decode_q4_glds, dim3(p.workgroups), dim3(256), 0, stream, idx,
                         (const float4*)p_loc, (const float4*)p_scale, p.qpb, p.bpw, nb,
                         (int64_t)1 << n_bits, rho, seed, block_id_base, (float4*)out_sample);
      break;
    case DecodeKernel::Q4:
      hipLaunchKernelGGL(k_decode_q4, dim3(p.workgroups), dim3(256), 0, stream, idx,
                         (const float4*)p_loc, (const float4*)p_scale, p.qpb, p.bpw, nb, n_steps,
                         (int64_t)1 << n_bits, nst, sdiv, rho, seed, block_id_base,
                         (float4*)out_sample);
      break;
    case DecodeKernel::General:
      hipLaunchKernelGGL(k_decode, dim3(p.workgroups), dim3(256), 0, stream, idx, p_loc, p_scale,
                         block_off, ud, nb, n_steps, (int64_t)1 << n_bits, nst, sdiv, rho, seed,
                         block_id_base, out_sample);
      break;
  }
  return hipGetLastError();
}

hipError_t launch_decode_csr_q4(const int32_t* idx, const int64_t* block_off,
                                const int64_t* slot_off, int64_t nb, int64_t n_slots,
                                const int32_t* block_seeds, int n_bits, int n_steps, float rho,
                                const float* dst_loc, const float* dst_scale, float* out,
                                hipStream_t stream) {
  if (nb <= 0 || n_slots <= 0) return hipSuccess;
  const int64_t grid = ((n_slots + 62) / 63 + 3) / 4;
  if (grid > 0x7fffffff) return hipErrorInvalidValue;
  const float nst = (float)n_steps;
  const float sdiv = (float)__builtin_sqrt((double)n_steps);
  hipLaunchKernelGGL(n_steps > 1 ? k_decode_csr_q4<2> : k_decode_csr_q4<1>, dim3((unsigned)grid),
                     dim3(256), 0, stream, idx, block_off,
                     slot_off, nb, n_slots, SeedSpec{0, 0, block_seeds}, n_steps,
                     (int64_t)1 << n_bits, nst, sdiv, rho, dst_loc, dst_scale, out);
  return hipGetLastError();
}

hipError_t launch_stateless_normal_sample(const float* loc, const float* scale, int64_t d,
                                          int64_t num_samples, int32_t seed, float* out,
                                          hipStream_t stream) {
  const int64_t total = d * num_samples;
  if (total <= 0) return hipSuccess;
  hipLaunchKernelGGL(k_stateless_normal_sample, dim3(grid_for((total + 3) / 4, 256, 65536)),
                     dim3(256), 0, stream, loc, scale, d, total, seed, out);
  return hipGetLastError();
}

hipError_t launch_standardise(const float* q_loc, const float* q_scale, const float* p_loc,
// ... 137 lines not shown
```

### compression_without_quantization_amd/csrc/cwq_workspace.h

```cpp
#pragma once
#include <stddef.h>
#include <stdint.h>

#include "cwq_dispatch.h"

#ifndef CWQ_CSR_GTAU_STRIDE
#define CWQ_CSR_GTAU_STRIDE 1
#endif
#define CWQ_SLIST_PER_BLOCK 8

namespace cwq {

constexpr int kTileQueueSlots = 64;
inline int64_t csr_rec_entries(int64_t total_dims) {
  return total_dims + 12 * (total_dims / (CWQ_CSR_LDS_DIMS + 1) + 1);
}
constexpr int kVbThreads = 256;
constexpr int kVbPerThread = 8;
constexpr int kVbTile = kVbThreads * kVbPerThread;
constexpr int kVbBins = 32;
constexpr int kVbcFactsRow = 2 * kVbBins + 2;
constexpr size_t kVbcFactsBytes = 1032;
inline int64_t vb_tiles(int64_t nb) { return (nb + kVbTile - 1) / kVbTile; }
constexpr int kPartW = 1024;
constexpr int kPartSuper = 256;
constexpr size_t kBatchItemBytes = 80;

struct Region {
  size_t off, bytes;
};
struct Arena {
  size_t o = 0;
  static size_t up(size_t v) { return (v + 255) / 256 * 256; }
  Region take(size_t bytes) {
    const Region r{o, bytes};
    o = up(o + bytes);
    return r;
  }
  Region take_packed(size_t bytes) {
    const Region r{o, bytes};
    o += bytes;
    return r;
  }
  Region take(const Arena& inner) { return take(inner.o - o); }
};
template <class T>
inline T* at(void* base, const Region& r) {
  return (T*)((char*)base + r.off);
}

struct EncWs {
  Region keys, tq, loc_s, scale_s, lognorm, slist, sab, cdim, bpre, ordu, grp, gtau, sdmap, abp;
  size_t total;
  bool screen;
  bool recs;
};
inline EncWs enc_ws(int64_t nb, int64_t total_dims, bool screen, bool recs) {
  EncWs l;
  Arena a;
  const size_t n = (size_t)nb, D = (size_t)total_dims;
  l.screen = screen;
  l.recs = screen && recs;
  l.keys = a.take(n * 8);
  l.tq = a.take((size_t)kTileQueueSlots * 4);
  l.loc_s = a.take(D * 4);
  l.scale_s = a.take(D * 4);
  l.lognorm = a.take(D * 4);
  l.slist = a.take(screen ? n * CWQ_SLIST_PER_BLOCK * 8 : 0);
  l.sab = a.take(screen ? (D + 8 * n + 4) * 8 : 0);
  l.cdim = a.take(screen ? D * 4 : 0);
  l.bpre = a.take(screen ? (D + 12 * n) * 4 : 0);
  l.ordu = a.take(screen ? (D + 12 * n) * 4 : 0);
  l.grp = a.take(screen ? n * 16 : 0);
  l.gtau = a.take(screen ? n * 4 * CWQ_CSR_GTAU_STRIDE : 0);
  l.sdmap = a.take(screen ? D * 4 : 0);
  l.abp = a.take(l.recs ? (size_t)csr_rec_entries(total_dims) * 32 : 0);
  l.total = a.o;
  return l;
}
inline EncWs enc_ws_csr(int64_t nb, int64_t total_dims, int64_t max_block_dim) {
  return enc_ws(nb, total_dims, has_screen_arrays(true, 0, nb),
                has_long_block_records(true, max_block_dim, nb));
}
inline EncWs enc_ws_uniform(int64_t nb, int64_t d) {
  return enc_ws(nb, nb * d, has_screen_arrays(false, d, nb), has_long_block_records(false, d, nb));
}

struct SortedWs {
  Region sorted_in, t_loc, t_scale, p_loc, p_scale;
  Region sample, seeds, perm, hist, counts;
  Region wgfacts, facts, soff, roff, src, partial;
};
inline SortedWs sorted_ws(Arena& a, bool csr, int64_t nb, int64_t total_dims) {
  SortedWs l{};
  const size_t n = (size_t)nb, row = (size_t)total_dims * 4, tiles = (size_t)vb_tiles(nb);
  Arena in{a.o};
  auto input = [&] { return csr ? a.take(row) : in.take_packed(row); };
  l.t_loc = input(), l.t_scale = input(), l.p_loc = input(), l.p_scale = input();
  if (!csr) l.sorted_in = a.take(in);
  l.sample = a.take(row);
  l.seeds = a.take(n * 4);
  l.perm = a.take(n * 4);
  l.hist = a.take(tiles * kVbBins * 4);
  l.counts = a.take(32 * 4);
  if (csr) {
    l.wgfacts = a.take(tiles * kVbcFactsRow * 8);
    l.facts = a.take(kVbcFactsBytes);
    l.soff = a.take((n + 1) * 8);
    l.roff = a.take((n + 33) * 8);
    l.src = a.take(n * 8);
    l.partial = a.take(tiles * 8);
  }
  return l;
}

struct VarWs {
  SortedWs s;
  Region enc, stage;
  size_t total;
  bool stage_aliases_sorted_in;
};
inline VarWs var_ws(int64_t nb, int64_t d, int64_t n_steps) {
  VarWs l;
  Arena a;
  l.s = sorted_ws(a, false, nb, nb * d);
  l.enc = a.take(enc_ws_uniform(nb, d).total);
  l.stage_aliases_sorted_in = n_steps <= 4 * d;
  const size_t stage = (size_t)nb * (size_t)n_steps * 4;
  l.stage = l.stage_aliases_sorted_in ? Region{l.s.sorted_in.off, stage} : a.take(stage);
  l.total = a.o;
  return l;
}

struct PackWs {
  Region off, partial, flag;
  size_t total;
};
inline PackWs pack_ws(int64_t nb) {
  PackWs l;
  Arena a;
  l.off = a.take((size_t)(nb + 1) * 8);
  l.partial = a.take((size_t)vb_tiles(nb) * 8);
  l.flag = a.take(4);
  l.total = a.o;
  return l;
}

inline VarWs var_csr_ws(int64_t nb, int64_t total_dims, int64_t max_block_dim, int64_t n_steps) {
  VarWs l{};
  Arena a;
  l.s = sorted_ws(a, true, nb, total_dims);
  l.stage = a.take((size_t)nb * (size_t)n_steps * 4);
  l.enc = a.take(enc_ws_csr(nb, total_dims, max_block_dim).total);
  l.total = a.o;
  return l;
}

struct PartWs {
  Region nxt, exg, node, gnode, conv, cnt, sup, spare;
  size_t total;
};
inline PartWs part_ws(int64_t D) {
  PartWs l;
  Arena a;
  const int64_t nch = (D + kPartW - 1) / kPartW, nsup = (nch + kPartSuper - 1) / kPartSuper;
  l.nxt = a.take_packed((size_t)(D + 64) * 4);
  l.exg = a.take_packed((size_t)(D + 64) * 4);
  l.node = a.take_packed((size_t)(D + 64) * 4);
// ... 261 lines not shown
```

### include/cwq.h

```cpp
#ifndef CWQ_H_
#define CWQ_H_

#include <stddef.h>
#include <stdint.h>

#ifdef __cplusplus
extern "C" {
#endif

#define CWQ_OK 0
#define CWQ_ERR_INVALID (-1)
#define CWQ_ERR_HIP (-2)
#define CWQ_ERR_WORKSPACE (-3)
#define CWQ_ERR_CAPACITY (-4)
#define CWQ_ERR_ALLOC (-5)

#define CWQ_MAX_BITS_PER_STEP 30

#define CWQ_ABI_VERSION ((0 << 16) | 15)
int cwq_version(void);

const char* cwq_last_error(void);

int cwq_stateless_normal_sample(const float* loc, const float* scale, int64_t d,
                                int64_t num_samples, int32_t seed, float* out, void* stream);

typedef struct cwq_options {
  int32_t prune_mode;
  int32_t reserved;
  void* eval_start_event;
  void* eval_stop_event;
  float* eval_ms_out;
  int32_t* item_ready;
} cwq_options;
#define CWQ_OPTIONS_INIT {2, 0, NULL, NULL, NULL, NULL}

size_t cwq_greedy_encode_workspace_size(int64_t nb, int64_t total_dims, int64_t max_block_dim);

size_t cwq_greedy_encode_uniform_workspace_size(int64_t nb, int64_t d);

int cwq_greedy_encode(const float* t_loc, const float* t_scale, const float* p_loc,
                      const float* p_scale, const int64_t* block_off, int64_t nb,
                      int64_t total_dims, int64_t max_block_dim, int n_bits_per_step,
                      int n_steps, int32_t seed, float rho, int64_t block_id_base,
                      int32_t* out_idx, float* out_sample, void* workspace,
                      size_t workspace_bytes, const cwq_options* opts, void* stream);

int cwq_greedy_encode_uniform(const float* t_loc, const float* t_scale, const float* p_loc,
                              const float* p_scale, int64_t nb, int64_t d,
                              int n_bits_per_step, int n_steps, int32_t seed, float rho,
                              int64_t block_id_base, int32_t* out_idx, float* out_sample,
                              void* workspace, size_t workspace_bytes, const cwq_options* opts,
                              void* stream);

int cwq_greedy_decode(const int32_t* idx, const float* p_loc, const float* p_scale,
                      const int64_t* block_off, int64_t nb, int64_t total_dims,
                      int64_t max_block_dim, int n_bits_per_step, int n_steps, int32_t seed,
                      float rho, int64_t block_id_base, float* out_sample, void* stream);

int cwq_greedy_decode_uniform(const int32_t* idx, const float* p_loc, const float* p_scale,
                              int64_t nb, int64_t d, int n_bits_per_step, int n_steps,
                              int32_t seed, float rho, int64_t block_id_base, float* out_sample,
                              void* stream);

int cwq_block_bits(const float* q_loc, const float* q_scale, const float* p_loc,
                   const float* p_scale, int64_t nb, int64_t d, double extra_bits, int min_bits,
                   int max_bits, int32_t* bits_out, float* kl_bits_out, void* stream);

size_t cwq_greedy_encode_uniform_var_workspace_size(int64_t nb, int64_t d);
int cwq_greedy_encode_uniform_var(const float* t_loc, const float* t_scale, const float* p_loc,
                                  const float* p_scale, int64_t nb, int64_t d,
                                  const int32_t* n_bits, int n_steps, int32_t seed, float rho,
                                  int64_t block_id_base, int32_t* out_idx, float* out_sample,
                                  void* workspace, size_t workspace_bytes,
                                  const cwq_options* opts, void* stream);

int cwq_block_bits_csr(const float* q_loc, const float* q_scale, const float* p_loc,
                       const float* p_scale, const int64_t* block_off, int64_t nb,
                       int64_t total_dims, double extra_bits, int n_steps, int min_bits,
                       int max_bits, int32_t* bits_out, float* kl_bits_out, void* stream);

size_t cwq_greedy_encode_var_workspace_size(int64_t nb, int64_t total_dims, int64_t max_block_dim,
                                            int n_steps);
int cwq_greedy_encode_var(const float* t_loc, const float* t_scale, const float* p_loc,
                          const float* p_scale, const int64_t* block_off, int64_t nb,
                          int64_t total_dims, int64_t max_block_dim, const int32_t* n_bits,
                          int n_steps, int32_t seed, float rho, int64_t block_id_base,
                          int32_t* out_idx, float* out_sample, void* workspace,
                          size_t workspace_bytes, const cwq_options* opts, void* stream);

size_t cwq_pack_indices_var_workspace_size(int64_t nb);
int cwq_pack_indices_var(const int32_t* idx, const int32_t* n_bits, int64_t nb, int n_steps,
                         uint8_t* out_bytes, int64_t out_cap, int64_t* total_bits_dev,
                         void* workspace, size_t workspace_bytes, void* stream);
int cwq_unpack_indices_var(const uint8_t* bytes, int64_t n_bytes, const int32_t* n_bits,
                           int64_t nb, int n_steps, int32_t* idx_out, void* workspace,
                           size_t workspace_bytes, void* stream);

int cwq_standardise(const float* q_loc, const float* q_scale, const float* p_loc,
                    const float* p_scale, int64_t n, float* t_loc, float* t_scale, void* stream);

int cwq_kl_normal_normal(const float* q_loc, const float* q_scale, const float* p_loc,
// ... 48 lines not shown
                          void* stream);

int cwq_importance_decode(const int64_t* index, const float* p_loc, const float* p_scale,
                          const int64_t* block_off, int64_t nb, int64_t total_dims, int32_t seed,
                          int64_t block_id_base, float* out_sample, void* stream);

int64_t cwq_importance_group_starts(const float* kl, int64_t D, int64_t size_threshold,
                                    double n_nats, int64_t* starts, int64_t cap);

int cwq_importance_plan(const float* kl, const int64_t* starts, int64_t ng, int64_t* n_samples);

size_t cwq_code_grouped_importance_workspace_size(int64_t D);
int64_t cwq_code_grouped_importance(const float* q_loc, const float* q_scale,
                                    const float* p_loc, const float* p_scale, int64_t D,
                                    int32_t seed, float dim_kl_bit_limit, int64_t size_threshold,
                                    double n_nats, float* sample_host, int64_t* index_host,
                                    int64_t* starts_host, int64_t starts_cap,
                                    int64_t* outlier_idx_host, float* outlier_val_host,
                                    int64_t* n_outliers, double* kl_sum_out, void* workspace,
                                    size_t workspace_bytes, const cwq_options* opts,
                                    void* stream);

size_t cwq_code_grouped_importance_batch_workspace_size(int64_t D_total, int64_t n_items);
int64_t cwq_code_grouped_importance_batch(
    int64_t n_items, const int64_t* item_off, const float* q_loc, const float* q_scale,
    const float* p_loc, const float* p_scale, const int32_t* seeds, float dim_kl_bit_limit,
    int64_t size_threshold, double n_nats, float* sample_host, int64_t* index_host,
    int64_t* starts_host, int64_t starts_cap, int64_t* n_starts, int64_t* outlier_idx_host,
    float* outlier_val_host, int64_t* n_outliers, double* kl_sum_out, void* workspace,
    size_t workspace_bytes, const cwq_options* opts, void* stream);

size_t cwq_decode_grouped_greedy_batch_workspace_size(int64_t D_total, int64_t G_total,
                                                      int n_steps);
size_t cwq_decode_grouped_greedy_batch_host_workspace_size(int64_t D_total, int64_t G_total,
                                                           int n_steps);
int64_t cwq_decode_grouped_greedy_batch(
    int64_t n_items, const int64_t* item_off, const float* p_loc, const float* p_scale,
    const char* bits_host, const int64_t* bits_off, const int64_t* starts_host,
    const int64_t* starts_off, int n_steps, int n_bits_per_step, const int32_t* seeds, float rho,
    float* sample_host, float* sample_dev, void* workspace, size_t workspace_bytes,
    void* host_workspace, size_t host_workspace_bytes, const cwq_options* opts, void* stream);

size_t cwq_decode_grouped_importance_batch_workspace_size(int64_t D_total, int64_t G_total);
size_t cwq_decode_grouped_importance_batch_host_workspace_size(int64_t D_total, int64_t G_total);
int64_t cwq_decode_grouped_importance_batch(
    int64_t n_items, const int64_t* item_off, const float* p_loc, const float* p_scale,
    const int64_t* index_host, const int64_t* index_off, const int64_t* starts_host,
    const int64_t* starts_off, const int32_t* seeds, float* sample_host, float* sample_dev,
    void* workspace, size_t workspace_bytes, void* host_workspace, size_t host_workspace_bytes,
    const cwq_options* opts, void* stream);

int64_t cwq_ac_encode(const int64_t* counts, int64_t K, int precision, const int64_t* message,
                      int64_t n, char* out_bits, int64_t cap);

int64_t cwq_ac_decode(const int64_t* counts, int64_t K, int precision, const char* bits,
                      int64_t nbits, int64_t* out_msg, int64_t cap);

int64_t cwq_elias_delta_encode(const int64_t* x, int64_t n, char* out, int64_t cap);
int64_t cwq_elias_delta_decode(const char* bits, int64_t nbits, int64_t count, int64_t* out);

int64_t cwq_bitcode_to_indices(const char* bits, int64_t nbits, int num_bits, int64_t count,
                               int32_t* out);

int cwq_selftest_bm_tables(uint32_t m0, int64_t count, float* radius, float* sin_out,
                           float* cos_out, void* stream);
int cwq_selftest_logf(const float* x, int64_t n, float* out, void* stream);
int cwq_selftest_screen_tables(uint32_t m0, int64_t count, float* radius, float* sin_out,
                               float* cos_out, void* stream);
int cwq_selftest_div(const float* a, const float* b, int64_t n, float* out, void* stream);
int cwq_selftest_wave_max(const float* x, int64_t n_waves, float* out, void* stream);
int cwq_selftest_encode_rows_wave(const float* t_loc, const float* t_scale, const float* p_loc,
                                  const float* p_scale, const int64_t* block_off, int64_t nb,
                                  int64_t total_dims, int64_t max_block_dim, int n_bits_per_step,
                                  int n_steps, int32_t seed, float rho, int64_t block_id_base,
                                  int32_t* out_idx, float* out_sample, void* workspace,
                                  size_t workspace_bytes, void* stream);
int cwq_selftest_encode_uniform_tau_guess(const float* t_loc, const float* t_scale,
                                          const float* p_loc, const float* p_scale, int64_t nb,
                                          int64_t d, int n_bits_per_step, int n_steps,
                                          int32_t seed, float rho, int64_t block_id_base,
                                          int32_t* out_idx, float* out_sample, void* workspace,
                                          size_t workspace_bytes, const cwq_options* opts,
                                          void* stream, int guess_mode);

#define CWQ_MAX_BEAM 16
size_t cwq_beam_encode_workspace_size(int64_t nb, int64_t total_dims, int64_t max_block_dim,
                                      int n_steps, int beam);
int cwq_beam_encode(const float* t_loc, const float* t_scale, const float* p_loc,
                    const float* p_scale, const int64_t* block_off, int64_t nb,
                    int64_t total_dims, int64_t max_block_dim, int n_bits_per_step, int n_steps,
                    int beam, int32_t seed, float rho, int64_t block_id_base, int32_t* out_idx,
                    float* out_sample, float* out_value, void* workspace, size_t workspace_bytes,
                    const cwq_options* opts, void* stream);
int cwq_selftest_beam_encode(const float* t_loc, const float* t_scale, const float* p_loc,
                             const float* p_scale, const int64_t* block_off, int64_t nb,
                             int64_t total_dims, int64_t max_block_dim, int n_bits_per_step,
                             int n_steps, int beam, int32_t seed, float rho,
                             int64_t block_id_base, int32_t* out_idx, float* out_sample,
                             float* out_value, void* workspace, size_t workspace_bytes,
                             const cwq_options* opts, void* stream, int path);

int cwq_beam_encode_var(const float* t_loc, const float* t_scale, const float* p_loc,
                        const float* p_scale, const int64_t* block_off, int64_t nb,
                        int64_t total_dims, int64_t max_block_dim, const int32_t* n_bits,
                        int max_bits, int n_steps, int beam, int32_t seed, float rho,
                        int64_t block_id_base, int32_t* out_idx, float* out_sample,
                        float* out_value, void* workspace, size_t workspace_bytes,
                        const cwq_options* opts, void* stream);
int cwq_selftest_beam_encode_var(const float* t_loc, const float* t_scale, const float* p_loc,
                                 const float* p_scale, const int64_t* block_off, int64_t nb,
                                 int64_t total_dims, int64_t max_block_dim, const int32_t* n_bits,
                                 int max_bits, int n_steps, int beam, int32_t seed, float rho,
                                 int64_t block_id_base, int32_t* out_idx, float* out_sample,
                                 float* out_value, void* workspace, size_t workspace_bytes,
                                 const cwq_options* opts, void* stream, int path);

#define CWQ_MAX_BACKFIT_SWEEPS 16
size_t cwq_greedy_backfit_workspace_size(int64_t nb, int64_t total_dims, int64_t max_block_dim,
                                         int n_steps);
int cwq_greedy_backfit(const float* t_loc, const float* t_scale, const float* p_loc,
                       const float* p_scale, const int64_t* block_off, int64_t nb,
                       int64_t total_dims, int64_t max_block_dim, int n_bits_per_step,
                       int n_steps, int sweeps, int32_t seed, float rho, int64_t block_id_base,
                       int32_t* idx_inout, float* out_sample, float* out_value,
                       int32_t* out_accepted, void* workspace, size_t workspace_bytes,
                       const cwq_options* opts, void* stream);

int cwq_greedy_backfit_var(const float* t_loc, const float* t_scale, const float* p_loc,
                           const float* p_scale, const int64_t* block_off ,
                           int64_t nb, int64_t total_dims, int64_t max_block_dim,
                           const int32_t* n_bits ,
                           int n_steps, int sweeps, int32_t seed, float rho,
                           int64_t block_id_base, int32_t* idx_inout, float* out_sample,
                           float* out_value, int32_t* out_accepted, void* workspace,
                           size_t workspace_bytes, const cwq_options* opts, void* stream);



int cwq_pln_posterior(const float* lik_loc, const float* lik_scale, const float* prior_loc,
                      const float* prior_scale, int64_t n, float eps, float* loc, float* scale,
                      void* stream);

int cwq_permute_gather(const float* src, int64_t C, int64_t HW, const int32_t* perm, float* out,
                       void* stream);

int cwq_permute_scatter(const float* src, int64_t C, int64_t HW, const int32_t* perm, float* out,
                        void* stream);

#ifdef __cplusplus
}
#endif
#endif
```

Before: 3.977 million.

## Defer full scoring: screen tiles first, score few survivors, rerun overflowed blocks

Splits the pruned encode into three launches. A screen-only pass runs one tile per block at higher occupancy and records up to Q survivors per block. A small kernel then scores those survivors across the whole batch, and a fallback pass fully processes only the blocks whose survivor list overflowed or was not produced. The aim is to stop each workgroup doing serialized per-tile survivor scoring and to raise waves per SIMD, at the cost of extra workspace, two extra launches and atomic bookkeeping. It is enabled by default for the uniform path when the work size reaches a threshold.

```diff
diff --git a/compression_without_quantization_amd/_lib.py b/compression_without_quantization_amd/_lib.py
--- a/compression_without_quantization_amd/_lib.py
+++ b/compression_without_quantization_amd/_lib.py
@@ -128,6 +128,10 @@
     "cwq_selftest_encode_uniform_tau_guess": (c_int, [c_vp, c_vp, c_vp, c_vp, c_i64, c_i64, c_int,
                                                       c_int, c_i32, c_f32, c_i64, c_vp, c_vp, c_vp,
                                                       c_size, c_opts, c_vp, c_int]),
+    "cwq_greedy_encode_uniform_defer_bytes": (c_size, [c_i64, c_i64]),
+    "cwq_selftest_encode_uniform_defer": (c_int, [c_vp, c_vp, c_vp, c_vp, c_i64, c_i64, c_int,
+                                                  c_int, c_i32, c_f32, c_i64, c_vp, c_vp, c_vp,
+                                                  c_size, c_opts, c_vp, c_int]),
     "cwq_beam_encode_workspace_size": (c_size, [c_i64, c_i64, c_i64, c_int, c_int]),
     "cwq_beam_encode": (c_int, [c_vp, c_vp, c_vp, c_vp, c_vp, c_i64, c_i64, c_i64, c_int, c_int,
                                 c_int, c_i32, c_f32, c_i64, c_vp, c_vp, c_vp, c_vp, c_size, c_opts,
@@ -162,7 +166,7 @@
                                               c_vp, c_vp]),
 }
 
-ABI_VERSION = (0 << 16) | 15
+ABI_VERSION = (0 << 16) | 16
 
 _lib = None
 
diff --git a/compression_without_quantization_amd/coded_greedy_sampler.py b/compression_without_quantization_amd/coded_greedy_sampler.py
--- a/compression_without_quantization_amd/coded_greedy_sampler.py
+++ b/compression_without_quantization_amd/coded_greedy_sampler.py
@@ -68,7 +68,7 @@
 def encode_workspace_bytes(nb, total_dims, block_dim=None, max_block_dim=None):
     lib = _lib.load()
     if block_dim is not None:
-        return int(lib.cwq_greedy_encode_uniform_workspace_size(int(nb), int(block_dim)))
+        return int(lib.cwq_greedy_encode_uniform_defer_bytes(int(nb), int(block_dim)))
     mbd = int(total_dims if max_block_dim is None else max_block_dim)
     return int(lib.cwq_greedy_encode_workspace_size(int(nb), int(total_dims), mbd))
 
diff --git a/compression_without_quantization_amd/csrc/cwq_capi.hip b/compression_without_quantization_amd/csrc/cwq_capi.hip
--- a/compression_without_quantization_amd/csrc/cwq_capi.hip
+++ b/compression_without_quantization_amd/csrc/cwq_capi.hip
@@ -298,7 +298,7 @@
                 void* workspace, size_t workspace_bytes, const cwq_options* opts, void* stream,
                 const int32_t* block_seeds = nullptr, float* ds_out = nullptr,
                 const float* ds_loc = nullptr, const float* ds_scale = nullptr,
-                bool rows_wave = false, int tau_guess = -1) {
+                bool rows_wave = false, int tau_guess = -1, int defer_mode = -2) {
   int rc = check_common(n_bits, n_steps, nb);
   if (rc) return rc;
   cwq_options o;
@@ -320,6 +320,22 @@
   a.ds_scale = ds_scale;
   a.rows_wave = rows_wave;
   a.tau_guess = tau_guess;
+  if (defer_mode >= -1 && !block_off) {
+    const cwq::DeferWs dl = cwq::defer_ws(l.total, nb, ud);
+    if (defer_mode >= 0 && (rc = check_ws(workspace, workspace_bytes, dl.total, NullWs::TakenIfEmpty)))
+      return rc;
+    if (dl.surv.bytes && workspace && workspace_bytes >= dl.total) {
+      a.defer_surv = at<uint32_t>(workspace, dl.surv);
+      a.defer_count = at<uint32_t>(workspace, dl.count);
+      a.defer_list = at<uint32_t>(workspace, dl.dlist);
+      a.defer_dcount = at<uint32_t>(workspace, dl.dcount);
+      a.defer_mode = defer_mode;
+    }
+    if (defer_mode >= 0 && dl.surv.bytes) {
+      a.tiles_per_block = 1;
+      a.cand_per_tile = (a.n_cand + 255) / 256 * 256;
+    }
+  }
   hipError_t e = cwq::launch_encode(a, (hipStream_t)stream);
   if (e != hipSuccess) return hip_fail(e, "cwq_greedy_encode");
   return ok();
@@ -435,6 +451,11 @@
   return cwq::enc_ws_uniform(nb, d).total;
 }
 
+size_t cwq_greedy_encode_uniform_defer_bytes(int64_t nb, int64_t d) {
+  if (nb < 0 || d < 0 || (d > 0 && nb > INT64_MAX / d)) return 0;
+  return cwq::defer_ws_uniform(nb, d).total;
+}
+
 int cwq_greedy_encode(const float* t_loc, const float* t_scale, const float* p_loc,
                       const float* p_scale, const int64_t* block_off, int64_t nb,
                       int64_t total_dims, int64_t max_block_dim, int n_bits_per_step,
@@ -458,7 +479,8 @@
   if (nb < 0 || (d > 0 && nb > INT64_MAX / d)) return fail(CWQ_ERR_INVALID, "bad nb");
   return encode_impl(t_loc, t_scale, p_loc, p_scale, nullptr, d, nb, nb * d, d, n_bits_per_step,
                      n_steps, seed, rho, block_id_base, out_idx, out_sample, workspace,
-                     workspace_bytes, opts, stream);
+                     workspace_bytes, opts, stream, nullptr, nullptr, nullptr, nullptr,
+                     false, -1, -1);
 }
 
 int cwq_greedy_decode(const int32_t* idx, const float* p_loc, const float* p_scale,
@@ -2675,6 +2697,22 @@
                      false, guess_mode);
 }
 
+int cwq_selftest_encode_uniform_defer(const float* t_loc, const float* t_scale,
+                                      const float* p_loc, const float* p_scale, int64_t nb,
+                                      int64_t d, int n_bits_per_step, int n_steps, int32_t seed,
+                                      float rho, int64_t block_id_base, int32_t* out_idx,
+                                      float* out_sample, void* workspace, size_t workspace_bytes,
+                                      const cwq_options* opts, void* stream, int defer_mode) {
+  if (d < 0) return fail(CWQ_ERR_INVALID, "d must be >= 0");
+  if (nb < 0 || (d > 0 && nb > INT64_MAX / d)) return fail(CWQ_ERR_INVALID, "bad nb");
+  if (defer_mode < 0 || defer_mode > 3)
+    return fail(CWQ_ERR_INVALID, "defer_mode=%d outside [0, 3]", defer_mode);
+  return encode_impl(t_loc, t_scale, p_loc, p_scale, nullptr, d, nb, nb * d, d, n_bits_per_step,
+                     n_steps, seed, rho, block_id_base, out_idx, out_sample, workspace,
+                     workspace_bytes, opts, stream, nullptr, nullptr, nullptr, nullptr,
+                     false, -1, defer_mode);
+}
+
 namespace {
 int beam_impl(const float* t_loc, const float* t_scale, const float* p_loc, const float* p_scale,
               const int64_t* block_off, int64_t nb, int64_t total_dims, int64_t max_block_dim,
diff --git a/compression_without_quantization_amd/csrc/cwq_kernels.h b/compression_without_quantization_amd/csrc/cwq_kernels.h
--- a/compression_without_quantization_amd/csrc/cwq_kernels.h
+++ b/compression_without_quantization_amd/csrc/cwq_kernels.h
@@ -38,6 +38,11 @@
   float* out_sample;
   unsigned long long* keys;
   uint32_t* tq = nullptr;
+  uint32_t* defer_surv = nullptr;
+  uint32_t* defer_count = nullptr;
+  uint32_t* defer_list = nullptr;
+  uint32_t* defer_dcount = nullptr;
+  int defer_mode = -1;
   float* loc_s;
   float* scale_s;
   float* lognorm;
diff --git a/compression_without_quantization_amd/csrc/cwq_kernels.hip b/compression_without_quantization_amd/csrc/cwq_kernels.hip
--- a/compression_without_quantization_amd/csrc/cwq_kernels.hip
+++ b/compression_without_quantization_amd/csrc/cwq_kernels.hip
@@ -95,6 +95,9 @@
 #ifndef CWQ_PRUNE_MIN_WAVES
 #define CWQ_PRUNE_MIN_WAVES 6
 #endif
+#ifndef CWQ_DEFER_MIN_WAVES
+#define CWQ_DEFER_MIN_WAVES 8
+#endif
 #ifndef CWQ_XCD_BALANCE
 #define CWQ_XCD_BALANCE 1
 #endif
@@ -161,6 +164,39 @@
 };
 static_assert(sizeof(VisitRec) == 48, "VisitRec: 48 bytes");
 
+template <int D, bool STEP0>
+__device__ __forceinline__ void score_block_terms(
+    const PhiloxStream& st, uint32_t row, uint32_t u, const float* __restrict__ loc_s,
+    const float* __restrict__ scale_s, const float* __restrict__ mu,
+    const float* __restrict__ sg, const float* __restrict__ lognorm,
+    const float* __restrict__ best, const double* logtab, float* rowterms) {
+  constexpr uint32_t G = D / 4;
+  const F4 z = normal4_dev(st, (uint64_t)row * G + u, logtab);
+#pragma unroll
+  for (int t = 0; t < 4; ++t) {
+    const uint32_t j = 4u * u + (uint32_t)t;
+    const float zz = t == 0 ? z.a : (t == 1 ? z.b : (t == 2 ? z.c : z.d));
+    float v = scale_s[j] * zz;
+    v = loc_s[j] + v;
+    const float tv = STEP0 ? v : best[j] + v;
+    rowterms[j] = log_prob(tv, mu[j], sg[j], lognorm[j]);
+  }
+}
+template <int D>
+__device__ __forceinline__ float score_fold8(const float* buf, uint32_t lane, bool valid) {
+  __builtin_amdgcn_fence(__ATOMIC_SEQ_CST, "wavefront");
+  __builtin_amdgcn_wave_barrier();
+  float acc = 0.0f;
+  const uint32_t fr = lane >> 3;
+  if (valid)
+    for (uint32_t e = lane & 7u; e < (uint32_t)D; e += 8u) acc = acc + buf[fr * D + e];
+  __builtin_amdgcn_fence(__ATOMIC_SEQ_CST, "wavefront");
+  __builtin_amdgcn_wave_barrier();
+  float p[8];
+#pragma unroll
+  for (int l = 0; l < 8; ++l) p[l] = __shfl(acc, (int)((lane & ~7u) + (uint32_t)l), 64);
+  return eigen_fold8(p, 0.0f);
+}
 template <int D, bool STEP0>
 __device__ __forceinline__ float score_rows_wave(
     const PhiloxStream& st, const uint32_t* rows, uint32_t cnt, const float* __restrict__ loc_s,
@@ -169,31 +205,22 @@
     const float* __restrict__ best, const double* logtab, float* buf, uint32_t lane) {
   constexpr uint32_t G = D / 4;
   const uint32_t r = lane / G, u = lane - r * G;
-  if (r < cnt) {
-    const F4 z = normal4_dev(st, (uint64_t)rows[r] * G + u, logtab);
-#pragma unroll
-    for (int t = 0; t < 4; ++t) {
-      const uint32_t j = 4u * u + (uint32_t)t;
-      const float zz = t == 0 ? z.a : (t == 1 ? z.b : (t == 2 ? z.c : z.d));
-      float v = scale_s[j] * zz;
-      v = loc_s[j] + v;
-      const float tv = STEP0 ? v : best[j] + v;
-      buf[r * D + j] = log_prob(tv, mu[j], sg[j], lognorm[j]);
-    }
-  }
-  __builtin_amdgcn_fence(__ATOMIC_SEQ_CST, "wavefront");
-  __builtin_amdgcn_wave_barrier();
-  float acc = 0.0f;
-  const uint32_t fr = lane >> 3;
-  if (fr < cnt)
-    for (uint32_t e = lane & 7u; e < (uint32_t)D; e += 8u) acc = acc + buf[fr * D + e];
-  __builtin_amdgcn_fence(__ATOMIC_SEQ_CST, "wavefront");
-  __builtin_amdgcn_wave_barrier();
-  float p[8];
-#pragma unroll
-  for (int l = 0; l < 8; ++l) p[l] = __shfl(acc, (int)((lane & ~7u) + (uint32_t)l), 64);
-  return eigen_fold8(p, 0.0f);
-}
+  if (r < cnt)
+    score_block_terms<D, STEP0>(st, rows[r], u, loc_s, scale_s, mu, sg, lognorm, best, logtab,
+                                buf + r * D);
+  return score_fold8<D>(buf, lane, (lane >> 3) < cnt);
+}
+
+template <int FORM>
+struct DeferArgs {
+  uint32_t* surv;
+  uint32_t* count;
+  uint32_t* list;
+  uint32_t* dcount;
+  int q;
+};
+template <>
+struct DeferArgs<0> {};
 
 #ifdef CWQ_TILE_TIMES
 constexpr int kTileTimes = 1 << 18;
@@ -241,16 +268,18 @@
   (f(std::integral_constant<uint32_t, I>{}, std::integral_constant<uint32_t, (uint32_t)sizeof...(I)>{}), ...);
 }
 
-template <int D, bool STEP0, bool INTER, bool PARK>
-__global__ void __launch_bounds__(256, CWQ_PRUNE_MIN_WAVES) k_encode_prune(
+template <int D, bool STEP0, bool INTER, bool PARK, int FORM = 0>
+__global__ void __launch_bounds__(256, FORM == 1 ? CWQ_DEFER_MIN_WAVES : CWQ_PRUNE_MIN_WAVES)
+k_encode_prune(
     const float* __restrict__ t_loc, const float* __restrict__ t_scale,
     const float* __restrict__ loc_s, const float* __restrict__ scale_s,
-    const float* __restrict__ lognorm, const float* __restrict__ best, int64_t ntiles,
+    const float* __restrict__ lognorm, const float* __restrict__ best, int64_t ntiles_arg,
     int64_t tiles_per_block, int64_t cand_per_tile, int64_t n_cand, SeedSpec sd, int32_t step,
     int allow_screen, unsigned long long* __restrict__ keys, int64_t tail_from, int tail_div,
-    uint32_t* __restrict__ tq) {
+    uint32_t* __restrict__ tq, DeferArgs<FORM> df) {
   static_assert(D % 8 == 0 && D >= 8 && D <= 64, "pruned path: D % 8 == 0, D <= 64");
   static_assert(!PARK || CWQ_PARK_COMPLETE, "PARK instances exist in CWQ_PARK_COMPLETE builds only");
+  static_assert(FORM == 0 || !INTER, "deferral: one tile per block");
   constexpr int G = D / 4;
   constexpr int NF = STEP0 ? 6 : 7;
   constexpr int RW = (64 / G) < 8 ? (64 / G) : 8;
@@ -281,7 +310,13 @@
   __shared__ uint32_t s_ps[72];
   for (int i = threadIdx.x; i < 72; i += blockDim.x) s_ps[i] = 0u;
 #endif
-  fill_logtab(logtab);
+  __shared__ uint32_t dq_cnt;
+  if constexpr (FORM != 1) fill_logtab(logtab);
+  int64_t ntiles = ntiles_arg;
+  if constexpr (FORM == 2) {
+    ntiles = (int64_t)__builtin_amdgcn_readfirstlane((int)*df.dcount);
+    if (ntiles > ntiles_arg) ntiles = ntiles_arg;
+  }
   const uint32_t wv = wave_id();
   const uint32_t lane = threadIdx.x & 63u;
 
@@ -309,8 +344,12 @@
     if (inter && CWQ_XCD_BALANCE && tq == nullptr && tile < treg && (treg & 7) == 0 &&
         (gridDim.x & 7u) == 0)
       tord = (tile & 7) * (treg >> 3) + (tile >> 3);
-    const int64_t g = inter ? tord % nbt : tile / tiles_per_block;
-    const int64_t tt = inter ? tord / nbt : tile - g * tiles_per_block;
+    int64_t g = inter ? tord % nbt : tile / tiles_per_block;
+    int64_t tt = inter ? tord / nbt : tile - g * tiles_per_block;
+    if constexpr (FORM == 2) {
+      g = (int64_t)(uint32_t)__builtin_amdgcn_readfirstlane((int)df.list[tile]);
+      tt = 0;
+    }
     const int64_t off = g * D;
     int64_t n0, csz;
     if (tt < tail_from) {
@@ -399,7 +438,8 @@
     }
     const bool fastdiv = __syncthreads_and(den_ok) != 0;
     const bool scr_all = __syncthreads_and(scr_ok) != 0;
-    const bool screen = (allow_screen & 1) && scr_all;
+    bool screen = (allow_screen & 1) && scr_all;
+    if constexpr (FORM == 1) screen = screen && df.q >= 0;
     if (wv == 1u) {
       const int gmode = (allow_screen >> 1) & 3;
       float qm = cwq::kTauNoGuess;
@@ -665,7 +705,7 @@
             if (slot < CWQ_SURVIVOR_CAP) {
               sq_n[slot] = (uint32_t)n;
               sq_ub[slot] = upper;
-            } else {
+            } else if constexpr (FORM != 1) {
 #ifdef CWQ_PRUNE_STATS
               atomicAdd(&g_prune_stats[69], 1ull);
 #endif
@@ -796,57 +836,86 @@
         __syncthreads();
         tau = (INTER && CWQ_TAU_FROM_KEYS) ? seed : -__builtin_inff();
       }
+    } else if constexpr (FORM == 1) {
+      tau_final = tau;
     } else {
       pass(std::false_type{});
       tau_share_wave(&tau_cell, tau);
       __syncthreads();
       tau_final = tau_cell;
     }
-    const uint32_t nsurv = sq_cnt < CWQ_SURVIVOR_CAP ? sq_cnt : CWQ_SURVIVOR_CAP;
-    const uint32_t nsurv_u = (uint32_t)__builtin_amdgcn_readfirstlane((int)nsurv);
-    const uint32_t sl = tid & 63u;
-    for (uint32_t c0 = wv * 64u; c0 < nsurv_u; c0 += 256u) {
-      const uint32_t i = c0 + sl;
-      const bool q = i < nsurv_u && sq_ub[i] >= tau_final;
-      const uint32_t nn = i < nsurv_u ? sq_n[i] : 0u;
-      const uint64_t qm = __builtin_amdgcn_ballot_w64(q);
-      if (qm == 0ull) continue;
+    if constexpr (FORM == 1) {
+      const uint32_t pushed = sq_cnt;
+      const bool listed = screen && pushed <= (uint32_t)CWQ_SURVIVOR_CAP;
+      const uint32_t qmax = df.q > 0 ? (uint32_t)df.q : 0u;
+      if (tid == 0) dq_cnt = 0u;
+      __syncthreads();
+      if (listed) {
+        for (uint32_t i = tid; i < pushed; i += 256u) {
+          if (sq_ub[i] >= tau_final) {
+            const uint32_t slot = atomicAdd(&dq_cnt, 1u);
+            if (slot < qmax) df.surv[cwq::defer_slot(g, (int)slot)] = sq_n[i];
+          }
+        }
+      }
+      __syncthreads();
+      if (tid == 0) {
+        const uint32_t c = dq_cnt;
+        const bool deferred = !listed || c > qmax;
+        df.count[g] = deferred ? 0u : cwq::defer_count_word(c, (int)qmax);
+        if (deferred) {
+          const uint32_t at = atomicAdd(df.dcount, 1u);
+          if ((int64_t)at < ntiles_arg) df.list[at] = (uint32_t)g;
+        }
+      }
+      __syncthreads();
+    } else {
+      const uint32_t nsurv = sq_cnt < CWQ_SURVIVOR_CAP ? sq_cnt : CWQ_SURVIVOR_CAP;
+      const uint32_t nsurv_u = (uint32_t)__builtin_amdgcn_readfirstlane((int)nsurv);
+      const uint32_t sl = tid & 63u;
+      for (uint32_t c0 = wv * 64u; c0 < nsurv_u; c0 += 256u) {
+        const uint32_t i = c0 + sl;
+        const bool q = i < nsurv_u && sq_ub[i] >= tau_final;
+        const uint32_t nn = i < nsurv_u ? sq_n[i] : 0u;
+        const uint64_t qm = __builtin_amdgcn_ballot_w64(q);
+        if (qm == 0ull) continue;
 #ifdef CWQ_PRUNE_STATS
-      if (q) atomicAdd(&g_prune_stats[68], 1ull);
-#endif
-      const uint32_t qr = __builtin_amdgcn_mbcnt_hi((uint32_t)(qm >> 32),
-                                                    __builtin_amdgcn_mbcnt_lo((uint32_t)qm, 0u));
-      __builtin_amdgcn_fence(__ATOMIC_SEQ_CST, "wavefront");
-      __builtin_amdgcn_wave_barrier();
-      if (q) sq_n[c0 + qr] = nn;
-      __builtin_amdgcn_fence(__ATOMIC_SEQ_CST, "wavefront");
-      __builtin_amdgcn_wave_barrier();
-      const uint32_t qn = (uint32_t)__builtin_popcountll(qm);
-      for (uint32_t b = 0; b < qn; b += (uint32_t)RW) {
-        const uint32_t cnt = qn - b < (uint32_t)RW ? qn - b : (uint32_t)RW;
-        const float v = score_rows_wave<D, STEP0>(
-            st, sq_n + c0 + b, cnt, loc_s + off, scale_s + off, t_loc + off, t_scale + off,
-            lognorm + off, STEP0 ? nullptr : best + off, logtab, rowbuf[wv], sl);
-        if ((sl & 7u) == 0u && (sl >> 3) < cnt) {
-          const uint64_t kv = argmax_key(v, sq_n[c0 + b + (sl >> 3)]);
-          bestk = kv > bestk ? kv : bestk;
-        }
-      }
-    }
-
-    bestk = wave_max_u64(bestk);
-    if (lane == 0) wkey[wv] = bestk;
-    __syncthreads();
-    if (tid == 0) {
-      uint64_t mk = wkey[0];
-      for (int i = 1; i < 4; ++i) mk = wkey[i] > mk ? wkey[i] : mk;
-      if (mk) atomicMax(&keys[g], (unsigned long long)mk);
+        if (q) atomicAdd(&g_prune_stats[68], 1ull);
+#endif
+        const uint32_t qr = __builtin_amdgcn_mbcnt_hi((uint32_t)(qm >> 32),
+                                                      __builtin_amdgcn_mbcnt_lo((uint32_t)qm, 0u));
+        __builtin_amdgcn_fence(__ATOMIC_SEQ_CST, "wavefront");
+        __builtin_amdgcn_wave_barrier();
+        if (q) sq_n[c0 + qr] = nn;
+        __builtin_amdgcn_fence(__ATOMIC_SEQ_CST, "wavefront");
+        __builtin_amdgcn_wave_barrier();
+        const uint32_t qn = (uint32_t)__builtin_popcountll(qm);
+        for (uint32_t b = 0; b < qn; b += (uint32_t)RW) {
+          const uint32_t cnt = qn - b < (uint32_t)RW ? qn - b : (uint32_t)RW;
+          const float v = score_rows_wave<D, STEP0>(
+              st, sq_n + c0 + b, cnt, loc_s + off, scale_s + off, t_loc + off, t_scale + off,
+              lognorm + off, STEP0 ? nullptr : best + off, logtab, rowbuf[wv], sl);
+          if ((sl & 7u) == 0u && (sl >> 3) < cnt) {
+            const uint64_t kv = argmax_key(v, sq_n[c0 + b + (sl >> 3)]);
+            bestk = kv > bestk ? kv : bestk;
+          }
+        }
+      }
+
+      bestk = wave_max_u64(bestk);
+      if (lane == 0) wkey[wv] = bestk;
+      __syncthreads();
+      if (tid == 0) {
+        uint64_t mk = wkey[0];
+        for (int i = 1; i < 4; ++i) mk = wkey[i] > mk ? wkey[i] : mk;
+        if (mk) atomicMax(&keys[g], (unsigned long long)mk);
 #ifdef CWQ_PRUNE_STATS
-      if (!g_seed_tau && g < kDbgBlocks) g_dbg_best[g] = mk;
+        if (!g_seed_tau && g < kDbgBlocks) g_dbg_best[g] = mk;
 #endif
 #ifdef CWQ_TILE_TIMES
-      if (tile < kTileTimes) g_tile_t1[tile] = __builtin_amdgcn_s_memrealtime();
-#endif
+        if (tile < kTileTimes) g_tile_t1[tile] = __builtin_amdgcn_s_memrealtime();
+#endif
+      }
     }
 #ifdef CWQ_PRUNE_STATS
     if (tid < 72) {
@@ -855,6 +924,49 @@
     }
 #endif
     __syncthreads();
+  }
+}
+
+__global__ void k_defer_reset(uint32_t* __restrict__ dcount) {
+  if (threadIdx.x == 0) *dcount = 0u;
+}
+
+template <int D, bool STEP0>
+__global__ void __launch_bounds__(256) k_score_survivors(
+    const float* __restrict__ t_loc, const float* __restrict__ t_scale,
+    const float* __restrict__ loc_s, const float* __restrict__ scale_s,
+    const float* __restrict__ lognorm, const float* __restrict__ best, int64_t nb, SeedSpec sd,
+    int32_t step, const uint32_t* __restrict__ surv, const uint32_t* __restrict__ count,
+    unsigned long long* __restrict__ keys) {
+  constexpr uint32_t G = D / 4;
+  constexpr uint32_t RW = (64 / G) < 8 ? (64 / G) : 8;
+  __shared__ double logtab[32];
+  __shared__ float rowbuf[4][RW * D];
+  fill_logtab(logtab);
+  const uint32_t wv = wave_id();
+  const uint32_t lane = threadIdx.x & 63u;
+  const int64_t g0 = ((int64_t)blockIdx.x * 4 + wv) * RW;
+  const uint32_t r = lane / G, u = lane - r * G, fr = lane >> 3;
+  const int64_t g = g0 + r, gf = g0 + fr;
+  const bool term_lane = r < RW && g < nb, fold_lane = fr < RW && gf < nb;
+  uint32_t cnt = term_lane ? count[g] : 0u, cntf = fold_lane ? count[gf] : 0u;
+  cnt = cnt < (uint32_t)cwq::kDeferSlots ? cnt : (uint32_t)cwq::kDeferSlots;
+  cntf = cntf < (uint32_t)cwq::kDeferSlots ? cntf : (uint32_t)cwq::kDeferSlots;
+  if (__builtin_amdgcn_ballot_w64(cnt != 0u) == 0ull) return;
+  PhiloxStream st{};
+  if (cnt != 0u) st = generate_key(step_seed(sd.of(g), step), 42);
+  const int64_t off = g * D;
+  for (uint32_t q = 0; q < (uint32_t)cwq::kDeferSlots; ++q) {
+    if (__builtin_amdgcn_ballot_w64(q < cnt) == 0ull) break;
+    if (q < cnt)
+      score_block_terms<D, STEP0>(st, surv[cwq::defer_slot(g, (int)q)], u, loc_s + off,
+                                  scale_s + off, t_loc + off, t_scale + off, lognorm + off,
+                                  STEP0 ? nullptr : best + off, logtab, rowbuf[wv] + r * D);
+    const float v = score_fold8<D>(rowbuf[wv], lane, q < cntf);
+    if ((lane & 7u) == 0u && q < cntf) {
+      const uint64_t kv = argmax_key(v, surv[cwq::defer_slot(gf, (int)q)]);
+      if (kv) atomicMax(&keys[gf], (unsigned long long)kv);
+    }
   }
 }
 
@@ -3024,7 +3136,7 @@
                        dim3((unsigned)(nt_s < kPruneGrid ? nt_s : kPruneGrid)), dim3(256), 0,
                        stream, a.t_loc, a.t_scale, a.loc_s, a.scale_s, a.lognorm, a.out_sample,
                        nt_s, seed_n / cpt_s, cpt_s, seed_n, seeds_of(a), step,
-                       prune_screen_arg(a), a.keys, seed_n / cpt_s, 1, nullptr);
+                       prune_screen_arg(a), a.keys, seed_n / cpt_s, 1, nullptr, DeferArgs<0>{});
   }
 #ifndef CWQ_TILE_QUEUE
 #define CWQ_TILE_QUEUE 1
@@ -3035,16 +3147,28 @@
 #ifndef CWQ_QUEUE_MIN_CPT
 #define CWQ_QUEUE_MIN_CPT 4096
 #endif
+#ifndef CWQ_DEFER
+#define CWQ_DEFER 1
+#endif
+#ifndef CWQ_DEFER_MIN_WORK
+#define CWQ_DEFER_MIN_WORK (1LL << 36)
+#endif
+  const int64_t tile_rows = a.cand_per_tile < a.n_cand ? a.cand_per_tile : a.n_cand;
+  bool defer = CWQ_DEFER && a.defer_surv && a.defer_count && a.defer_list && a.defer_dcount &&
+               a.defer_mode != 0 && (prune_screen_arg(a) & 1) && a.tiles_per_block == 1 &&
+               !seeded && ntiles < (1LL << 31) &&
+               (a.defer_mode >= 1 || ntiles >= (CWQ_DEFER_MIN_WORK + tile_rows * D - 1) / (tile_rows * D));
+  if (defer) hipLaunchKernelGGL(k_defer_reset, dim3(1), dim3(64), 0, stream, a.defer_dcount);
+  const int64_t queue_grid = defer ? 256 * (int64_t)CWQ_DEFER_MIN_WAVES : (int64_t)CWQ_QUEUE_GRID;
   uint32_t* tq = nullptr;
   if (CWQ_TILE_QUEUE && a.tq != nullptr && ntiles < (1LL << 31) &&
-      a.cand_per_tile >= CWQ_QUEUE_MIN_CPT && ntiles > CWQ_QUEUE_GRID) {
+      a.cand_per_tile >= CWQ_QUEUE_MIN_CPT && ntiles > queue_grid) {
     if (hipMemsetAsync(a.tq, 0, sizeof(uint32_t), stream) == hipSuccess) tq = a.tq;
   }
   auto qgrid = [&](int64_t nt) -> unsigned {
-    const int64_t cap = tq ? (int64_t)CWQ_QUEUE_GRID : kPruneGrid;
+    const int64_t cap = tq ? queue_grid : kPruneGrid;
     return (unsigned)(nt < cap ? nt : cap);
   };
-  const int64_t tile_rows = a.cand_per_tile < a.n_cand ? a.cand_per_tile : a.n_cand;
   auto with_park = [&](auto launch) {
     if constexpr (CWQ_PARK_COMPLETE && D >= CWQ_PARK_MIN_D) {
       if (tile_rows * D >= (int64_t)CWQ_PARK_MIN_ROWS * 32) return launch(std::true_type{});
@@ -3070,7 +3194,32 @@
                          dim3(qgrid(nt2)), dim3(256), 0,
                          stream, a.t_loc, a.t_scale, a.loc_s, a.scale_s, a.lognorm, a.out_sample,
                          nt2, tpb2, a.cand_per_tile, a.n_cand, seeds_of(a), step,
-                         prune_screen_arg(a), a.keys, from, (int)div, tq);
+                         prune_screen_arg(a), a.keys, from, (int)div, tq, DeferArgs<0>{});
+    });
+  } else if (defer) {
+    const int q = a.defer_mode == 2 ? -1 : (a.defer_mode == 3 ? 0 : (int)kDeferQ);
+    static_assert(kDeferQ >= 0 && kDeferQ <= kDeferSlots, "Q slots per block");
+    with_park([&](auto park) {
+      hipLaunchKernelGGL((k_encode_prune<D, STEP0, false, decltype(park)::value, 1>),
+                         dim3(qgrid(ntiles)), dim3(256), 0,
+                         stream, a.t_loc, a.t_scale, a.loc_s, a.scale_s, a.lognorm, a.out_sample,
+                         ntiles, a.tiles_per_block, a.cand_per_tile, a.n_cand, seeds_of(a), step,
+                         prune_screen_arg(a), a.keys, a.tiles_per_block, 1, tq,
+                         DeferArgs<1>{a.defer_surv, a.defer_count, a.defer_list, a.defer_dcount, q});
+    });
+    constexpr int64_t kRowsPerWg = 4 * ((64 / (D / 4)) < 8 ? (64 / (D / 4)) : 8);
+    hipLaunchKernelGGL((k_score_survivors<D, STEP0>),
+                       dim3((unsigned)((a.nb + kRowsPerWg - 1) / kRowsPerWg)), dim3(256), 0, stream,
+                       a.t_loc, a.t_scale, a.loc_s, a.scale_s, a.lognorm, a.out_sample, a.nb,
+                       seeds_of(a), step, (const uint32_t*)a.defer_surv,
+                       (const uint32_t*)a.defer_count, a.keys);
+    with_park([&](auto park) {
+      hipLaunchKernelGGL((k_encode_prune<D, STEP0, false, decltype(park)::value, 2>),
+                         dim3((unsigned)(ntiles < 1536 ? ntiles : 1536)), dim3(256), 0,
+                         stream, a.t_loc, a.t_scale, a.loc_s, a.scale_s, a.lognorm, a.out_sample,
+                         ntiles, a.tiles_per_block, a.cand_per_tile, a.n_cand, seeds_of(a), step,
+                         prune_screen_arg(a), a.keys, a.tiles_per_block, 1, nullptr,
+                         DeferArgs<2>{a.defer_surv, a.defer_count, a.defer_list, a.defer_dcount, q});
     });
   } else {
     with_park([&](auto park) {
@@ -3078,7 +3227,7 @@
                          dim3(qgrid(ntiles)), dim3(256), 0,
                          stream, a.t_loc, a.t_scale, a.loc_s, a.scale_s, a.lognorm, a.out_sample,
                          ntiles, a.tiles_per_block, a.cand_per_tile, a.n_cand, seeds_of(a), step,
-                         prune_screen_arg(a), a.keys, a.tiles_per_block, 1, tq);
+                         prune_screen_arg(a), a.keys, a.tiles_per_block, 1, tq, DeferArgs<0>{});
     });
   }
 }
@@ -3386,6 +3535,7 @@
     if (a.seeds) p.seeds = a.seeds + g0;
     p.keys = a.keys + g0;
     if (a.tq) p.tq = a.tq + i;
+    p.defer_surv = nullptr;
     p.out_idx = a.out_idx + g0 * a.n_steps;
     if (a.sab) p.sab = a.sab + 8 * g0;
     if (a.bpre) p.bpre = a.bpre + 12 * g0;
diff --git a/compression_without_quantization_amd/csrc/cwq_workspace.h b/compression_without_quantization_amd/csrc/cwq_workspace.h
--- a/compression_without_quantization_amd/csrc/cwq_workspace.h
+++ b/compression_without_quantization_amd/csrc/cwq_workspace.h
@@ -6,6 +6,9 @@
 
 #ifndef CWQ_CSR_GTAU_STRIDE
 #define CWQ_CSR_GTAU_STRIDE 1
+#endif
+#ifndef CWQ_DEFER_Q
+#define CWQ_DEFER_Q 2
 #endif
 #define CWQ_SLIST_PER_BLOCK 8
 
@@ -84,6 +87,32 @@
 }
 inline EncWs enc_ws_uniform(int64_t nb, int64_t d) {
   return enc_ws(nb, nb * d, has_screen_arrays(false, d, nb), has_long_block_records(false, d, nb));
+}
+
+constexpr int kDeferSlots = 4;
+constexpr int kDeferQ = CWQ_DEFER_Q;
+inline bool defer_shape(int64_t nb, int64_t d) {
+  return nb > 0 && nb < (1LL << 31) && d % 8 == 0 && d >= 8 && d <= 64;
+}
+constexpr size_t defer_slot(int64_t g, int q) { return (size_t)g * kDeferSlots + (size_t)q; }
+constexpr uint32_t defer_count_word(uint32_t c, int Q) { return c <= (uint32_t)Q ? c : 0u; }
+struct DeferWs {
+  Region surv, count, dlist, dcount;
+  size_t total;
+};
+inline DeferWs defer_ws(size_t enc_total, int64_t nb, int64_t d) {
+  DeferWs l;
+  Arena a{Arena::up(enc_total)};
+  const size_t n = defer_shape(nb, d) ? (size_t)nb : 0;
+  l.surv = a.take(n * kDeferSlots * 4);
+  l.count = a.take(n * 4);
+  l.dlist = a.take(n * 4);
+  l.dcount = a.take(n ? 4 : 0);
+  l.total = a.o;
+  return l;
+}
+inline DeferWs defer_ws_uniform(int64_t nb, int64_t d) {
+  return defer_ws(enc_ws_uniform(nb, d).total, nb, d);
 }
 
 struct SortedWs {
diff --git a/include/cwq.h b/include/cwq.h
--- a/include/cwq.h
+++ b/include/cwq.h
@@ -17,7 +17,7 @@
 
 #define CWQ_MAX_BITS_PER_STEP 30
 
-#define CWQ_ABI_VERSION ((0 << 16) | 15)
+#define CWQ_ABI_VERSION ((0 << 16) | 16)
 int cwq_version(void);
 
 const char* cwq_last_error(void);
@@ -232,6 +232,13 @@
                                           int32_t* out_idx, float* out_sample, void* workspace,
                                           size_t workspace_bytes, const cwq_options* opts,
                                           void* stream, int guess_mode);
+size_t cwq_greedy_encode_uniform_defer_bytes(int64_t nb, int64_t d);
+int cwq_selftest_encode_uniform_defer(const float* t_loc, const float* t_scale,
+                                      const float* p_loc, const float* p_scale, int64_t nb,
+                                      int64_t d, int n_bits_per_step, int n_steps, int32_t seed,
+                                      float rho, int64_t block_id_base, int32_t* out_idx,
+                                      float* out_sample, void* workspace, size_t workspace_bytes,
+                                      const cwq_options* opts, void* stream, int defer_mode);
 
 #define CWQ_MAX_BEAM 16
 size_t cwq_beam_encode_workspace_size(int64_t nb, int64_t total_dims, int64_t max_block_dim,
```

After: 4.034 million (median of 6 runs). 1.01x the previous value.
